# ethz-asl/TULIP

Hardware: AMD Instinct MI355X
Metric: range-images/sec training (KITTI 16->64x1024, bs=8/GPU) (higher is better)
Workload: dtype bf16; 1 GPU; tulip_base 16x1024->64x1024 training step (fwd+L1+bwd+allreduce+AdamW), per-GPU batch 8, window 2x8, patch 1x4, DropPath 0.1, reference init seed 0; global_batch=8, parallelism=dp1, hip_graph=True

## Files before the change

### include/tulip_hip.h

```cpp
#ifndef TULIP_HIP_H_
#define TULIP_HIP_H_

#include <stdint.h>

#ifdef __cplusplus
extern "C" {
#endif

#ifndef __HIP_PLATFORM_AMD__
typedef struct ihipStream_t* hipStream_t;
#endif

#define TULIP_EPI_BF16 0
#define TULIP_EPI_GELU_DUAL 1
#define TULIP_EPI_GELU_BWD 2
#define TULIP_EPI_F32 3
#define TULIP_EPI_RESID_F32 4
#define TULIP_EPI_PIXSHUF2_F32 5
#define TULIP_EPI_SPLIT_F32 7
#define TULIP_EPI_UNSHUF2_BF16 8

#define TULIP_GEMM_ACCUMULATE 1
#define TULIP_GEMM_NO_TOUCH 0x100
#define TULIP_GEMM_CHECKED 0x200
// ... 169 lines not shown
                           const float* gscale_dev, float gscale, hipStream_t stream, int in_chans, int r);
int tulip_tail_bwd_dgrad_ln_r(const uint16_t* xn, const uint16_t* We, const float* be, const float* wd, const float* dpred,
                              float* dwd_partials, int B, int H, int W, int E, const float* target, const float* gscale_dev,
                              float gscale, const float* x, const float* mean, const float* rstd, const float* gamma,
                              float* dx, uint16_t* dx_bf16, const float* cast_rowscale, int cast_rows_per_sample,
                              float* ln_partials, hipStream_t stream, int in_chans, int r);
int tulip_tail_fwd_ln_r(const float* x, const float* gamma, const float* beta, float eps, uint16_t* xn, float* mean,
                        float* rstd, const uint16_t* We, const float* be, const float* wd, float* pred, const float* target,
                        float* loss_partials, int log_transform, int B, int H, int W, int E, hipStream_t stream,
                        int in_chans, int r);
int tulip_tail_wgrad_splits_r(int B, int H, int W, int E, int in_chans, int r);
int tulip_tail_wgrad_r(const uint16_t* xn, const uint16_t* We, const float* be, const float* wd, const float* dpred,
                       float* slabs_w, float* slabs_b, int B, int H, int W, int E, const float* target,
                       const float* gscale_dev, float gscale, hipStream_t stream, int in_chans, int r);


int tulip_expand_norm_fwd(const float* y, const float* gamma, const float* beta, uint16_t* out_bf16, int ld,
                          const float* dotw, float* pred, float* mean, float* rstd, int B, int H, int W, int P, int Cn,
                          float eps, hipStream_t stream);
int tulip_expand_norm_bwd(const uint16_t* dy_fine, int ld, const float* dpred, const float* dotw, const float* y,
                          const float* mean, const float* rstd, const float* gamma, const float* beta, uint16_t* dy_nat,
                          float* partials, int B, int H, int W, int P, int Cn, hipStream_t stream);
int tulip_expand_norm_fwd_c(const float* y, const float* gamma, const float* beta, uint16_t* out_bf16, int ld,
                            const float* dotw, float* pred, float* mean, float* rstd, int B, int H, int W, int P, int Cn,
                            float eps, hipStream_t stream, int in_chans);
int tulip_expand_norm_bwd_c(const uint16_t* dy_fine, int ld, const float* dpred, const float* dotw, const float* y,
                            const float* mean, const float* rstd, const float* gamma, const float* beta, uint16_t* dy_nat,
                            float* partials, int B, int H, int W, int P, int Cn, hipStream_t stream, int in_chans);
int tulip_expand_norm_bwd_partial_rows(int B, int H, int W, int P);

int tulip_l1_loss_fwd(const float* pred, const float* target, float* partials, float* losses, int64_t n,
                      int log_transform, hipStream_t stream);
int tulip_l1_loss_bwd(const float* pred, const float* target, const float* gscale_dev, float gscale, float* dpred,
                      int64_t n, hipStream_t stream);

int tulip_adamw(float* p, float* g, float* m, float* v, uint16_t* p_bf16, int64_t n, const float* hyper,
                const uint8_t* decay_mask64, int zero_grad, hipStream_t stream);
int tulip_adamw_blocks(float* p, float* g, float* m, float* v, uint16_t* p_bf16, const int32_t* blocks, int nblocks,
                       const float* hyper, const uint8_t* decay_mask64, int zero_grad, hipStream_t stream);
int tulip_adamw_s(float* p, float* g, float* m, float* v, uint16_t* p_bf16, int64_t n, const float* hyper,
                  const uint8_t* decay_mask64, const float* lr_scale64, int zero_grad, hipStream_t stream);
int tulip_adamw_blocks_s(float* p, float* g, float* m, float* v, uint16_t* p_bf16, const int32_t* blocks, int nblocks,
                         const float* hyper, const uint8_t* decay_mask64, const float* lr_scale64, int zero_grad,
                         hipStream_t stream);

int tulip_drop_path_scales(const float* keep, float* scale, float* u_out, int nslots, int B, uint64_t seed,
                           uint64_t* counter, hipStream_t stream);

int tulip_dropout_begin(uint64_t* counter, uint64_t* key_out, int advance, hipStream_t stream);
int tulip_dropout_mask(const uint64_t* key_ptr, uint64_t seed, int site, float p, int64_t n, float* out, hipStream_t stream);
int tulip_dropout_scale(void* x, int is_bf16, int rows, int cols, int ld, const uint64_t* key_ptr, uint64_t seed, int site,
                        float p, hipStream_t stream);
int tulip_dropout_resid_ln(const float* y, const float* aux, const float* rowscale, int rows_per_sample, float* out,
                           uint16_t* out_bf16, const float* gamma, const float* beta, uint16_t* xn, float* mean, float* rstd,
                           float eps, int rows, int C, const uint64_t* key_ptr, uint64_t seed, int site, float p,
                           hipStream_t stream);
int tulip_dropout_cast(const float* dx, uint16_t* y, int rows, int cols, const float* rowscale, int rows_per_sample,
                       const uint64_t* key_ptr, uint64_t seed, int site, float p, hipStream_t stream);
int tulip_window_attn_fwd_drop(const uint16_t* qkv, const float* bias_table, const int32_t* rel_index, uint16_t* out, int B,
                               int H, int W, int C, int nh, int wh, int ww, int sh, int sw, int masked,
                               const uint64_t* key_ptr, uint64_t seed, int site, float p, hipStream_t stream);
int tulip_window_attn_bwd_drop(const uint16_t* qkv, const uint16_t* dout, const float* bias_table, const int32_t* rel_index,
                               uint16_t* dqkv, float* dbias_partials, int B, int H, int W, int C, int nh, int wh, int ww,
                               int sh, int sw, int masked, const uint64_t* key_ptr, uint64_t seed, int site, float p,
                               hipStream_t stream);

int tulip_grad_norm(const float* g, int64_t n, double* partials, const float* scale_dev, float scale, float* out,
                    hipStream_t stream);

int tulip_range_prep(const void* raw, int raw_dtype, int64_t batch_stride, int64_t row_stride, int64_t col_stride,
                     int64_t base_offset, float* hi, float* lo, int B, int H, int W, int row_factor, int col_factor,
                     int row_phase, int col_phase, float scale, int gate, float min_range, float max_range,
                     int log_transform, int roll_shift, hipStream_t stream);


int tulip_mc_aggregate(const float* preds, int passes, int64_t n, float noise_threshold, float* out,
                       hipStream_t stream);

int tulip_eval_postprocess(const float* pred, const float* hi, const float* lo, float* pred_img, float* hi_img,
                           double* partials, float* mae_out, int H, int W, int h, int w, int log_transform,
                           float gate_min, float gate_max, float keep_close, hipStream_t stream);

int tulip_range_to_xyz(const float* img, const float* sin_h, const float* cos_h, const float* sin_v,
                       const float* cos_v, float max_range, int H, int W, float* xyz, hipStream_t stream);

int tulip_range_to_xyz_durlar(const float* img, const double* col_tables, const double* row_tables,
                              const int32_t* row_offset, float max_range, float origin_offset, double z_offset, int H,
                              int W, double* xyz, hipStream_t stream);

int tulip_voxel_metrics(const void* pcd_pred, int64_t n_pred, const void* pcd_gt, int64_t n_gt, int is_f64,
                        double grid_size, uint32_t* bitmap_pred, uint32_t* bitmap_gt, int64_t bitmap_words,
                        double* scratch, double* out, hipStream_t stream);

int tulip_chamfer_sq(const void* a, int64_t na, const void* b, int64_t nb, int is_f64, float* dist_a, float* dist_b,
                     double* scratch, double* out, hipStream_t stream);

int tulip_kitti_range_map(const float* points, int64_t n, int rows, int cols, float ang_start_y, float ang_res_y,
                          float ang_res_x, float max_range, float min_range, int32_t* winner, float* out,
                          hipStream_t stream);

typedef struct tulip_swin96_desc {
    const float* x_in; float* x1; float* x_out;
    void* xn1; void* qkv; void* attn_out; void* xn2; void* fc1_pre; void* fc1_act;
    float* mean1; float* rstd1; float* mean2; float* rstd2;
    const void* w_qkv; const void* w_proj; const void* w_fc1; const void* w_fc2;
    const float* b_qkv; const float* b_proj; const float* b_fc1; const float* b_fc2;
    const float* norm1_weight; const float* norm1_bias; const float* norm2_weight; const float* norm2_bias;
    const float* bias_table; const int32_t* rel_index; const float* drop_scale_attn; const float* drop_scale_mlp;
    int B; int H; int W; int shift_h; int shift_w; int masked; float eps;
} tulip_swin96_desc;
int tulip_swin96_block_fwd(const tulip_swin96_desc* d, hipStream_t stream);
int tulip_swin96_block_fwd_profiled(const tulip_swin96_desc* d, uint64_t* stamps, hipStream_t stream);
int tulip_swin96_pair_sync_bytes(int B, int H, int W);
int tulip_swin96_pair_fwd(const tulip_swin96_desc* d0, const tulip_swin96_desc* d1, void* sync, size_t sync_bytes,
                          hipStream_t stream);

typedef struct tulip_swin96_bwd_desc {
    float* dx; const float* x_in; const float* x1;
    const void* qkv; const void* fc1_pre;
    const float* mean1; const float* rstd1; const float* mean2; const float* rstd2;
    const void* w_qkv; const void* w_proj; const void* w_fc1; const void* w_fc2;
    const float* norm1_weight; const float* norm2_weight;
    const float* bias_table; const int32_t* rel_index; const float* drop_scale_attn; const float* drop_scale_mlp;
    void* d_out_mlp; void* d_fc1_pre; void* d_out_attn; void* d_qkv;
    void* dx_bf16; const float* dx_bf16_scale;
    float* norm1_partials; float* norm2_partials; float* bias_partials;
    int B; int H; int W; int shift_h; int shift_w; int masked;
    const float* b_qkv; const float* b_fc1; const float* norm1_bias; const float* norm2_bias;
} tulip_swin96_bwd_desc;
int tulip_swin96_bwd_partial_rows(int B, int H, int W);
int tulip_swin96_block_bwd(const tulip_swin96_bwd_desc* d, hipStream_t stream);
int tulip_swin96_block_bwd_profiled(const tulip_swin96_bwd_desc* d, uint64_t* stamps, hipStream_t stream);

#define TULIP_PACK_MAX 64
typedef struct tulip_pack_item { const void* src; void* dst; int rows; int cols; int transpose; } tulip_pack_item;
int tulip_swinw_supported(int C, int H, int W);
int tulip_swinw_block_fwd(const tulip_swin96_desc* d, int C, void* out_bf16, hipStream_t stream);
int tulip_swinw_block_fwd_profiled(const tulip_swin96_desc* d, int C, void* out_bf16, uint64_t* stamps,
                                   hipStream_t stream);
int tulip_swinw_split_bytes(int C, int B, int H, int W);
int tulip_swinw_block_fwd_split(const tulip_swin96_desc* d, int C, void* out_bf16, void* exchange, size_t exchange_bytes,
                                uint64_t* stamps, hipStream_t stream);
int tulip_swinw_bwd_partial_rows(int C, int B, int H, int W);
int tulip_swinw_block_bwd(const tulip_swin96_bwd_desc* d, int C, hipStream_t stream);
int tulip_swinw_block_bwd_split(const tulip_swin96_bwd_desc* d, int C, void* exchange, size_t exchange_bytes, hipStream_t stream);
int tulip_pack_bf16_multi(const tulip_pack_item* items, int n, hipStream_t stream);

int tulip_swind_supported(int C, int H, int W, int wh, int ww);
int tulip_swind_groups(int C, int B, int H, int W, int wh, int ww);
int tulip_swind_block_fwd(const tulip_swin96_desc* d, int C, int wh, int ww, void* out_bf16, int phases, uint64_t* stamps,
                          hipStream_t stream);
int tulip_swind_block_bwd(const tulip_swin96_bwd_desc* d, int C, int wh, int ww, float* d_norm_out, int phases, uint64_t* stamps,
                          hipStream_t stream);


typedef struct tulip_merge_fwd_desc {
    const float* x; const float* gamma; const float* beta;
    const void* w_packed;
    void* xm; float* mean; float* rstd; float* y;
    void* y_bf16; int ld_bf16;
    int B, H, W, Cin; float eps;
} tulip_merge_fwd_desc;
int tulip_merge_fwd_supported(int Cin, int B, int H, int W);
int tulip_merge_fwd(const tulip_merge_fwd_desc* d, hipStream_t stream);

typedef struct tulip_merge_bwd_desc {
    const float* dx_in; const void* dy_skip; const void* w_skip_t_packed;
    void* dyb;
    const void* w_red_t_packed;
    const float* x_prev; const float* mean; const float* rstd; const float* gamma;
    float* dx_prev; float* param_partials;
    void* dx_bf16; const float* cast_rowscale; int cast_rows_per_sample;
    int B, H, W, Cp;
} tulip_merge_bwd_desc;
int tulip_merge_bwd_supported(int Cp, int B, int H, int W);
int tulip_merge_bwd_partial_rows(int Cp, int B, int H, int W);
int tulip_merge_bwd(const tulip_merge_bwd_desc* d, hipStream_t stream);

typedef struct tulip_unmerge_skip_desc {
    const void* x_bf16;
    const void* w_expand_packed; const float* b_expand;
    void* cat;
    const void* w_skip_packed; const float* b_skip;
    float* out;
    int B, H, W, C;
} tulip_unmerge_skip_desc;
int tulip_unmerge_skip_supported(int C, int B, int H, int W);
int tulip_unmerge_skip_fwd(const tulip_unmerge_skip_desc* d, hipStream_t stream);

typedef struct tulip_skip_unmerge_bwd_desc {
    const void* dy_skip; const void* w_skip_t_packed;
    void* dz;
    const void* w_expand_t_packed;
    float* dx; void* dx_bf16; const float* cast_rowscale; int cast_rows_per_sample;
    int B, H, W, C;
} tulip_skip_unmerge_bwd_desc;
int tulip_skip_unmerge_bwd(const tulip_skip_unmerge_bwd_desc* d, hipStream_t stream);

int tulip_stamp_realtime(uint64_t* dst, hipStream_t stream);
#define TULIP_ABI_VERSION 6
int tulip_abi_version(void);
const char* tulip_build_arch(void);
int tulip_dev_variants(void);

#ifdef __cplusplus
}
#endif
#endif
```

### tulip_amd/_lib.py

```python
from __future__ import annotations

import ctypes
import os
from ctypes import c_char_p, c_double, c_float, c_int, c_int64, c_void_p

_PKG = os.path.dirname(os.path.abspath(__file__))
LIB_PATH = os.environ.get("TULIP_HIP_LIB") or os.path.join(_PKG, "libtulip_hip.so")

P, I, F, L, D = c_void_p, c_int, c_float, c_int64, c_double

class Swin96Desc(ctypes.Structure):
    _fields_ = [(n, P) for n in ("x_in", "x1", "x_out", "xn1", "qkv", "attn_out", "xn2", "fc1_pre", "fc1_act", "mean1",
                                 "rstd1", "mean2", "rstd2", "w_qkv", "w_proj", "w_fc1", "w_fc2", "b_qkv", "b_proj",
                                 "b_fc1", "b_fc2", "norm1_weight", "norm1_bias", "norm2_weight", "norm2_bias",
                                 "bias_table", "rel_index", "drop_scale_attn", "drop_scale_mlp")] + \
               [(n, I) for n in ("B", "H", "W", "shift_h", "shift_w", "masked")] + [("eps", F)]


class Swin96BwdDesc(ctypes.Structure):
    _fields_ = [(n, P) for n in ("dx", "x_in", "x1", "qkv", "fc1_pre", "mean1", "rstd1", "mean2", "rstd2", "w_qkv",
                                 "w_proj", "w_fc1", "w_fc2", "norm1_weight", "norm2_weight", "bias_table", "rel_index",
                                 "drop_scale_attn", "drop_scale_mlp", "d_out_mlp", "d_fc1_pre", "d_out_attn", "d_qkv",
                                 "dx_bf16", "dx_bf16_scale", "norm1_partials", "norm2_partials", "bias_partials")] + \
               [(n, I) for n in ("B", "H", "W", "shift_h", "shift_w", "masked")] + \
               [(n, P) for n in ("b_qkv", "b_fc1", "norm1_bias", "norm2_bias")]


class ReduceRegion(ctypes.Structure):
    _fields_ = [("partials", P), ("out", P), ("stride", L), ("n", L), ("rows", I), ("overwrite", I),
                ("scatter_index", P), ("scatter_nh", I), ("scatter_len", I), ("adamw", I)]


class WgradItem(ctypes.Structure):
    _fields_ = [("dY", P), ("X", P), ("dW", P), ("db", P), ("ldy", I), ("ldx", I), ("Nw", I), ("Kw", I), ("Mtok", I),
                ("splits", I), ("overwrite", I), ("reserved_", I)]


class AdamwRef(ctypes.Structure):
    _fields_ = [(n, P) for n in ("hyper", "grad", "param", "exp_avg", "exp_avg_sq", "param_bf16", "decay_mask64")]


class DropDraw(ctypes.Structure):
    _fields_ = [("keep", P), ("scale", P), ("u_out", P), ("nslots", I), ("B", I), ("seed", ctypes.c_uint64), ("counter", P)]


class PackItem(ctypes.Structure):
    _fields_ = [("src", P), ("dst", P), ("rows", I), ("cols", I), ("transpose", I)]


class MergeFwdDesc(ctypes.Structure):
    _fields_ = [("x", P), ("gamma", P), ("beta", P), ("w_packed", P), ("xm", P), ("mean", P), ("rstd", P), ("y", P),
                ("y_bf16", P), ("ld_bf16", I), ("B", I), ("H", I), ("W", I), ("Cin", I), ("eps", F)]


class MergeBwdDesc(ctypes.Structure):
    _fields_ = [("dx_in", P), ("dy_skip", P), ("w_skip_t_packed", P), ("dyb", P), ("w_red_t_packed", P), ("x_prev", P),
                ("mean", P), ("rstd", P), ("gamma", P), ("dx_prev", P), ("param_partials", P), ("dx_bf16", P),
                ("cast_rowscale", P), ("cast_rows_per_sample", I), ("B", I), ("H", I), ("W", I), ("Cp", I)]


class UnmergeSkipDesc(ctypes.Structure):
    _fields_ = [("x_bf16", P), ("w_expand_packed", P), ("b_expand", P), ("cat", P), ("w_skip_packed", P), ("b_skip", P),
                ("out", P), ("B", I), ("H", I), ("W", I), ("C", I)]


class SkipUnmergeBwdDesc(ctypes.Structure):
    _fields_ = [("dy_skip", P), ("w_skip_t_packed", P), ("dz", P), ("w_expand_t_packed", P), ("dx", P), ("dx_bf16", P),
                ("cast_rowscale", P), ("cast_rows_per_sample", I), ("B", I), ("H", I), ("W", I), ("C", I)]


REDUCE_REGIONS_MAX, WGRAD_GROUP_MAX, PACK_MAX = 48, 16, 64
LR_GROUP_SHIFT, LR_GROUPS_MAX = 2, 64
GEMM_NO_TOUCH, GEMM_CHECKED, GEMM_NO_MID, GEMM_MID, WGRAD_SMALL_TILES, BLOCK_NO_WARM = 0x100, 0x200, 0x400, 0x800, 0x100, 8
GEMM_B_PACKED = 0x1000
ROUTE_TILE, ROUTE_FULL, ROUTE_MID, ROUTE_STREAM = range(4)
ROUTE_DEEP, ROUTE_A_TRANS, ROUTE_B_TRANS, ROUTE_FOLD, ROUTE_SPLITS_SHIFT = 0x10, 0x20, 0x40, 0x80, 8
ABI_VERSION = 6

SIGNATURES = {
    "tulip_gemm_bf16": [P, I, I, P, I, I, I, I, I, I, P, P, I, P, I, P, I, P, I, I, I, I, I, P, L, P],
    "tulip_swin96_block_fwd": [P, P],
    "tulip_swin96_pair_sync_bytes": [I, I, I],
    "tulip_swin96_pair_fwd": [P, P, P, ctypes.c_size_t, P],
    "tulip_swin96_block_bwd": [P, P],
    "tulip_swin96_block_fwd_profiled": [P, P, P],
    "tulip_swin96_block_bwd_profiled": [P, P, P],
    "tulip_swin96_bwd_partial_rows": [I, I, I],
    "tulip_swinw_supported": [I, I, I],
    "tulip_swinw_block_fwd": [P, I, P, P],
    "tulip_swinw_block_fwd_profiled": [P, I, P, P, P],
    "tulip_swinw_split_bytes": [I, I, I, I],
    "tulip_swinw_block_fwd_split": [P, I, P, P, ctypes.c_size_t, P, P],
    "tulip_swinw_bwd_partial_rows": [I, I, I, I],
    "tulip_swinw_block_bwd": [P, I, P],
    "tulip_swinw_block_bwd_split": [P, I, P, ctypes.c_size_t, P],
    "tulip_swind_supported": [I, I, I, I, I],
    "tulip_swind_groups": [I, I, I, I, I, I],
    "tulip_swind_block_fwd": [P, I, I, I, P, I, P, P],
    "tulip_swind_block_bwd": [P, I, I, I, P, I, P, P],
    "tulip_pack_bf16_multi": [P, I, P],
    "tulip_layernorm_fwd": [P, P, P, P, P, P, I, I, F, I, I, I, I, P],
    "tulip_layernorm_bwd": [P, P, P, P, P, P, P, I, I, I, I, I, I, P, P, P, I, P],
    "tulip_layernorm_bwd_splitk": [P, I, P, P, P, P, P, P, I, I, I, I, I, I, P, P, P, I, P],
    "tulip_splitk_resid_ln_supported": [I],
    "tulip_splitk_resid_ln": [P, I, I, I, P, P, I, P, I, P, I, P, I, P, P, P, P, P, F, P],
    "tulip_layernorm_bwd_partial_rows": [I, I],
    "tulip_layernorm_bwd_params": [P, P, P, P, P, P, I, I, I, I, I, I, P],
    "tulip_patch_embed_fwd": [P, P, P, P, P, P, I, I, I, I, I, I, I, I, I, F, P, I, P],
    "tulip_patch_embed_fwd_draw": [P, P, P, P, P, P, I, I, I, I, I, I, I, I, I, F, P, I, P, P],
    "tulip_patch_embed_bwd": [P, P, P, P, P, P, P, P, P, I, I, I, I, I, I, I, I, I, F, I, P],
    "tulip_patch_embed_bwd_blocks": [I],
    "tulip_window_attn_fwd": [P, P, P, P, I, I, I, I, I, I, I, I, I, I, P],
    "tulip_window_attn_bwd": [P, P, P, P, P, P, I, I, I, I, I, I, I, I, I, I, P],
    "tulip_window_attn_bwd_partial_rows": [I, I, I, I, I, I],
    "tulip_cast_f32_bf16": [P, P, I, I, P, I, P],
    "tulip_reduce_splits": [P, P, L, I, P],
    "tulip_reduce_rows2": [P, L, P, L, P, L, P, L, I, P],
    "tulip_reduce_rows_multi": [P, I, P],
    "tulip_reduce_rows_multi_adamw": [P, I, P, P],
    "tulip_wgrad_group": [P, I, P, I, P, L, I, P],
    "tulip_wgrad_tiles": [I, I, I],
    "tulip_wgrad_group_regions": [P, I, P, P, I],
    "tulip_wgrad_group_adamw": [P, I, P, I, P, L, I, P, P],
    "tulip_wgrad_group_profiled": [P, I, P, L, I, P, P],
    "tulip_gemm_effective_splits": [I, I],
    "tulip_gemm_packed_supported": [I, I, I, I],
    "tulip_gemm_route": [I, I, I, I, I, I, I, I],
    "tulip_cast_flat": [P, P, L, P],
    "tulip_cast_bf16_f32": [P, P, L, P],
    "tulip_tail_fwd": [P, P, P, P, P, I, I, I, I, P],
    "tulip_tail_bwd": [P, P, P, P, P, P, P, I, I, I, I, P, P, F, P],
    "tulip_tail_fused_bwd_supported": [I],
    "tulip_tail_bwd_dgrad": [P, P, P, P, P, P, P, I, I, I, I, P, P, F, P],
    "tulip_tail_bwd_dgrad_ln": [P, P, P, P, P, P, I, I, I, I, P, P, F, P, P, P, P, P, P, P, I, P, P],
    "tulip_tail_fwd_ln": [P, P, P, F, P, P, P, P, P, P, P, P, P, I, I, I, I, I, P],
    "tulip_l1_loss_final": [P, P, I, L, I, P],
    "tulip_tail_wgrad_splits": [I, I, I, I],
    "tulip_tail_wgrad": [P, P, P, P, P, P, P, I, I, I, I, P, P, F, P],
    "tulip_expand_norm_fwd": [P, P, P, P, I, P, P, P, P, I, I, I, I, I, F, P],
    "tulip_expand_norm_bwd": [P, I, P, P, P, P, P, P, P, P, P, I, I, I, I, I, P],
    "tulip_expand_norm_bwd_partial_rows": [I, I, I, I],
    "tulip_tail_fwd_c": [P, P, P, P, P, I, I, I, I, P, I],
    "tulip_tail_bwd_c": [P, P, P, P, P, P, P, I, I, I, I, P, P, F, P, I],
    "tulip_tail_bwd_dgrad_c": [P, P, P, P, P, P, P, I, I, I, I, P, P, F, P, I],
    "tulip_tail_bwd_dgrad_ln_c": [P, P, P, P, P, P, I, I, I, I, P, P, F, P, P, P, P, P, P, P, I, P, P, I],
    "tulip_tail_fwd_ln_c": [P, P, P, F, P, P, P, P, P, P, P, P, P, I, I, I, I, I, P, I],
    "tulip_tail_wgrad_c": [P, P, P, P, P, P, P, I, I, I, I, P, P, F, P, I],
    "tulip_tail_fwd_r": [P, P, P, P, P, I, I, I, I, P, I, I],
    "tulip_tail_bwd_r": [P, P, P, P, P, P, P, I, I, I, I, P, P, F, P, I, I],
    "tulip_tail_fused_bwd_supported_r": [I, I],
    "tulip_tail_bwd_dgrad_r": [P, P, P, P, P, P, P, I, I, I, I, P, P, F, P, I, I],
    "tulip_tail_bwd_dgrad_ln_r": [P, P, P, P, P, P, I, I, I, I, P, P, F, P, P, P, P, P, P, P, I, P, P, I, I],
    "tulip_tail_fwd_ln_r": [P, P, P, F, P, P, P, P, P, P, P, P, P, I, I, I, I, I, P, I, I],
    "tulip_tail_wgrad_splits_r": [I, I, I, I, I, I],
    "tulip_tail_wgrad_r": [P, P, P, P, P, P, P, I, I, I, I, P, P, F, P, I, I],
    "tulip_expand_norm_fwd_c": [P, P, P, P, I, P, P, P, P, I, I, I, I, I, F, P, I],
    "tulip_expand_norm_bwd_c": [P, I, P, P, P, P, P, P, P, P, P, I, I, I, I, I, P, I],
    "tulip_l1_loss_fwd": [P, P, P, P, L, I, P],
    "tulip_l1_loss_bwd": [P, P, P, F, P, L, P],
    "tulip_adamw": [P, P, P, P, P, L, P, P, I, P],
    "tulip_adamw_blocks": [P, P, P, P, P, P, I, P, P, I, P],
    "tulip_adamw_s": [P, P, P, P, P, L, P, P, P, I, P],
    "tulip_adamw_blocks_s": [P, P, P, P, P, P, I, P, P, P, I, P],
    "tulip_wgrad_group_adamw_s": [P, I, P, I, P, L, I, P, P, P],
    "tulip_reduce_rows_multi_adamw_s": [P, I, P, P, P],
    "tulip_drop_path_scales": [P, P, P, I, I, ctypes.c_uint64, P, P],
    "tulip_dropout_begin": [P, P, I, P],
    "tulip_dropout_mask": [P, ctypes.c_uint64, I, F, L, P, P],
    "tulip_dropout_scale": [P, I, I, I, I, P, ctypes.c_uint64, I, F, P],
    "tulip_dropout_resid_ln": [P, P, P, I, P, P, P, P, P, P, P, F, I, I, P, ctypes.c_uint64, I, F, P],
    "tulip_dropout_cast": [P, P, I, I, P, I, P, ctypes.c_uint64, I, F, P],
    "tulip_window_attn_fwd_drop": [P, P, P, P, I, I, I, I, I, I, I, I, I, I, P, ctypes.c_uint64, I, F, P],
    "tulip_window_attn_bwd_drop": [P, P, P, P, P, P, I, I, I, I, I, I, I, I, I, I, P, ctypes.c_uint64, I, F, P],
    "tulip_grad_norm": [P, L, P, P, F, P, P],
    "tulip_kitti_range_map": [P, L, I, I, F, F, F, F, F, P, P, P],
    "tulip_range_prep": [P, I, L, L, L, L, P, P, I, I, I, I, I, I, I, F, I, F, F, I, I, P],
    "tulip_mc_aggregate": [P, I, L, F, P, P],
    "tulip_eval_postprocess": [P, P, P, P, P, P, P, I, I, I, I, I, F, F, F, P],
    "tulip_range_to_xyz": [P, P, P, P, P, F, I, I, P, P],
    "tulip_range_to_xyz_durlar": [P, P, P, P, F, F, D, I, I, P, P],
    "tulip_voxel_metrics": [P, L, P, L, I, D, P, P, L, P, P, P],
    "tulip_chamfer_sq": [P, L, P, L, I, P, P, P, P, P],
    "tulip_merge_fwd_supported": [I, I, I, I],
    "tulip_merge_fwd": [P, P],
    "tulip_merge_bwd_supported": [I, I, I, I],
    "tulip_merge_bwd_partial_rows": [I, I, I, I],
    "tulip_merge_bwd": [P, P],
    "tulip_unmerge_skip_supported": [I, I, I, I],
    "tulip_unmerge_skip_fwd": [P, P],
    "tulip_skip_unmerge_bwd": [P, P],
    "tulip_stamp_realtime": [P, P],
    "tulip_abi_version": [],
    "tulip_build_arch": [],
    "tulip_dev_variants": [],
}

(EPI_BF16, EPI_GELU_DUAL, EPI_GELU_BWD, EPI_F32, EPI_RESID_F32, EPI_PIXSHUF2_F32, _EPI_RETIRED_6,
 EPI_SPLIT_F32, EPI_UNSHUF2_BF16) = range(9)

_lib = None


class TulipHipError(RuntimeError):
    pass


DEV_LIB_PATH = os.path.join(_PKG, "libtulip_hip_dev.so")
_libs = {}
_dev_depth = [1 if (os.environ.get("TULIP_HIP_DEV", "0") == "1" or os.environ.get("TULIP_SWIN96_RECOMPUTE", "0") != "0" or
                    os.environ.get("TULIP_SWINW_SPLIT_BWD", "0") != "0" or os.environ.get("TULIP_FC1_GRAD_WIDE", "1") == "0" or
                    os.environ.get("TULIP_FUSE_WIDE", "1") == "0") else 0]


def _open(path: str) -> ctypes.CDLL:
    if not os.path.exists(path):
        raise TulipHipError(
            f"{path} not found: build it with `python -m tulip_amd.csrc.build` "
            "(tulip_amd has no CPU or PyTorch fallback for the hot path)")
    import torch
    lib = ctypes.CDLL(path)
    for name, argtypes in SIGNATURES.items():
        try:
            fn = getattr(lib, name)
        except AttributeError as e:
            raise TulipHipError(f"symbol {name} missing from {path}") from e
        fn.argtypes = argtypes
        fn.restype = c_char_p if name == "tulip_build_arch" else c_int
    if lib.tulip_abi_version() != ABI_VERSION:
        raise TulipHipError(f"{path}: ABI version mismatch; rebuild")
    return lib


def load() -> ctypes.CDLL:
    global _lib
    path = DEV_LIB_PATH if _dev_depth[0] and not os.environ.get("TULIP_HIP_LIB") else LIB_PATH
    lib = _libs.get(path)
    if lib is None:
        lib = _libs[path] = _open(path)
    _lib = lib
    return lib


class dev_library:
    def __enter__(self):
        _dev_depth[0] += 1
        return load()

    def __exit__(self, *exc):
        _dev_depth[0] -= 1
        return False


# ... 13 lines not shown
```

### tulip_amd/csrc/swind.hip

```cpp
#ifndef TULIP_STORE_LATE_D
#define TULIP_STORE_LATE_D 1
#endif
#define TULIP_STORE_LATE TULIP_STORE_LATE_D
#include "common.h"
#include "tulip_hip.h"
#include "swin_stream.h"

namespace {

constexpr int NS = 8;

template <int C, int G>
struct GeoD {
    static constexpr int NH = C / 32, NWV = C / 128, NT = NWV * 64, T = 16 * G, KS = C / 32, HPW = NH / NS, HID = 4 * C;
    static constexpr int HS = HID / NS, KH = KS / 2, KSH = HS / 32;
    static constexpr int LPT = C / 48;
    static_assert(NWV == 2 * HPW && HS == 64 * NWV && C / 16 == 8 * NWV && (LPT == 16 || LPT == 32), "wave layout");
    static constexpr int XN_BYTES = T * C * 2;
    static constexpr int A_QX = XN_BYTES, A_QX_BYTES = HPW * 6 * G * 1024;
    static constexpr int A_HT = A_QX + A_QX_BYTES, A_HT_BYTES = HPW * 3072;
    static constexpr int A_AFF = A_HT + A_HT_BYTES;
    static constexpr int A_WARM = A_AFF + 8 * C;
    static constexpr int A_SMEM = A_WARM + 1024;
    static constexpr int B_AFF = XN_BYTES;
    static constexpr int B_WARM = B_AFF + 8 * C;
    static constexpr int B_SMEM = B_WARM + 1024;
    static constexpr int N_WARM = 2 * XN_BYTES;
    static constexpr int N_SMEM = N_WARM + 1024;
    static_assert(A_SMEM <= 163840 && N_SMEM <= 163840, "LDS");
};

struct TokMapD {
    int b, wy, wx0, H, W, wh, ww, lw, sh, sw;
    __device__ __forceinline__ void coords(int tt, int& hs, int& ws) const {
        const int t = tt & 15;
        hs = wy * wh + (t >> lw);
        ws = ((wx0 + (tt >> 4)) << lw) + (t & (ww - 1));
    }
    __device__ __forceinline__ size_t row(int tt) const {
        int hs, ws;
        coords(tt, hs, ws);
        int hh = hs + sh; if (hh >= H) hh -= H;
        int w2 = ws + sw; if (w2 >= W) w2 -= W;
        return ((size_t)b * H + hh) * W + w2;
    }
    __device__ __forceinline__ int label(int tt) const {
        int hs, ws;
        coords(tt, hs, ws);
        return 3 * region(hs, H, wh, sh) + region(ws, W, ww, sw);
    }
};
template <int G>
__device__ __forceinline__ TokMapD make_map_d(int H, int W, int wh, int ww, int sh, int sw, int grp) {
    const int nWx = W / ww, nWy = H / wh, gpr = nWx / G;
    TokMapD m;
    m.b = grp / (nWy * gpr);
    grp -= m.b * nWy * gpr;
    m.wy = grp / gpr;
    m.wx0 = (grp - m.wy * gpr) * G;
    m.H = H; m.W = W; m.wh = wh; m.ww = ww; m.lw = ww == 16 ? 4 : 3; m.sh = sh; m.sw = sw;
    return m;
}

template <int NTILE, int KSTEPS, int PF, int SEG = KSTEPS, int SEGSTRIDE = KSTEPS>
struct WS {
    bf16x8 ring[PF][NTILE];
    const bf16_t* wt[NTILE];
    static constexpr int koff(int p) { return 512 * ((p / SEG) * SEGSTRIDE + (p % SEG)); }
    __device__ __forceinline__ void start() {
        static_for<PF>([&](auto P_) {
            constexpr int p = decltype(P_)::value;
            if constexpr (p < KSTEPS) {
#pragma unroll
                for (int i = 0; i < NTILE; ++i) ring[p][i] = *(const bf16x8*)(wt[i] + koff(p));
            }
        });
    }
    template <int G, int T>
    __device__ __forceinline__ void run(f32x4 (&acc)[NTILE][G], const unsigned char* act, int t, int gq) {
        static_for<KSTEPS>([&](auto K_) {
            constexpr int ks = decltype(K_)::value;
            bf16x8 a[NTILE];
#pragma unroll
            for (int i = 0; i < NTILE; ++i) a[i] = ring[ks % PF][i];
            if constexpr (ks + PF < KSTEPS) {
#pragma unroll
                for (int i = 0; i < NTILE; ++i) ring[ks % PF][i] = *(const bf16x8*)(wt[i] + koff(ks + PF));
            }
            bf16x8 b[G];
#pragma unroll
            for (int g = 0; g < G; ++g) b[g] = frag<T>(act, ks, 16 * g + t, gq);
#pragma unroll
            for (int i = 0; i < NTILE; ++i)
#pragma unroll
                for (int g = 0; g < G; ++g) acc[i][g] = __builtin_amdgcn_mfma_f32_16x16x32_bf16(a[i], b[g], acc[i][g], 0, 0, 0);
        });
    }
};

struct SliceWarm {
    unsigned char* sink;
    int nslot, slot, ws, loff;
    bool on;
    __device__ __forceinline__ void init(int grp, int ngrp, int wid, int lane, unsigned char* lds_sink) {
        nslot = ngrp < 32 ? ngrp : 32; slot = grp; on = grp < 32;
        ws = __builtin_amdgcn_readfirstlane(wid); loff = lane * 16; sink = lds_sink;
    }
    template <int NWV>
    __device__ __forceinline__ void touch(const bf16_t* w, int nruns, int run, int stride) {
        if (!on) return;
        const int total = nruns * run;
        for (int c = slot * NWV + ws; c < total; c += nslot * NWV) {
            const int r = c / run, o = c - r * run;
            warm_touch16((const unsigned char*)(w + ((size_t)r * stride + o) * 512) + loff, sink);
        }
    }
};


struct DeepArgs {
    const float* xin; float* x1; float* xout;
    bf16_t *xn1, *qkv, *o, *xn2, *h, *g;
    float *mean1, *rstd1, *mean2, *rstd2;
    const bf16_t *wqkv, *wproj, *w1, *w2;
    const float *bqkv, *bproj, *b1, *b2, *g1, *be1, *g2, *be2;
    const float* bias_table; const int* rel_index;
    const float *ds0, *ds1;
    bf16_t* out_bf16;
    const float* dx;
    bf16_t *dyb_m, *dh, *dyb_a, *dqkv;
    float* dxn;
    float* biaspart;
    unsigned long long* prof;
    int B, H, W, wh, ww, sh, sw, masked, save, ngrp;
    float eps, scale;
};
#if TULIP_DEV_VARIANTS
#define DEEP_STAMP(k) do { if (a.prof && lane == 0) a.prof[((size_t)blockIdx.x * NWV + wid) * 16 + (k)] = __builtin_amdgcn_s_memtime(); } while (0)
#else
#define DEEP_STAMP(k) ((void)0)
#endif

template <int C, int T, int NWV>
struct RowPro {
    static constexpr int LPT = C / 48, TPW = 64 / LPT, NJ = 12, NP = (T + NWV * TPW - 1) / (NWV * TPW);
    float4 xv[NP][NJ];
    size_t row[NP];
    int tl;
    __device__ __forceinline__ int tok(int p, int wid, int lane) const { return wid * TPW + lane / LPT + p * NWV * TPW; }
    __device__ __forceinline__ void load(const float* __restrict__ x, const TokMapD& tm, int wid, int lane) {
        tl = lane % LPT;
#pragma unroll
        for (int p = 0; p < NP; ++p) {
            const int tt = tok(p, wid, lane);
            row[p] = tm.row(tt < T ? tt : T - 1);
            if (tt < T) {
#pragma unroll
                for (int j = 0; j < NJ; ++j) xv[p][j] = *(const float4*)(x + row[p] * C + 4 * tl + 4 * LPT * j);
            }
        }
    }
    __device__ __forceinline__ void layernorm(const float* aff, float eps, unsigned char* XN, bf16_t* save, float* mean, float* rstd,
                                              bool sv, int wid, int lane) {
#pragma unroll
        for (int p = 0; p < NP; ++p) {
            const int tt = tok(p, wid, lane);
            if (tt < T) {
                float sm = 0.f;
#pragma unroll
                for (int j = 0; j < NJ; ++j) sm += (xv[p][j].x + xv[p][j].y) + (xv[p][j].z + xv[p][j].w);
                const float mu = group_sum<LPT>(sm) * (1.0f / C);
                float q = 0.f;
#pragma unroll
                for (int j = 0; j < NJ; ++j) {
                    const float d0 = xv[p][j].x - mu, d1 = xv[p][j].y - mu, d2 = xv[p][j].z - mu, d3 = xv[p][j].w - mu;
                    q += (d0 * d0 + d1 * d1) + (d2 * d2 + d3 * d3);
                }
                const float rs = rsqrtf(group_sum<LPT>(q) * (1.0f / C) + eps);
                if (sv && tl == 0) { mean[row[p]] = mu; rstd[row[p]] = rs; }
#pragma unroll
                for (int j = 0; j < NJ; ++j) {
                    const int c = 4 * tl + 4 * LPT * j;
                    const float4 ga = *(const float4*)(aff + c), be = *(const float4*)(aff + C + c);
                    const bf16x4 pk = pack4((xv[p][j].x - mu) * rs * ga.x + be.x, (xv[p][j].y - mu) * rs * ga.y + be.y,
                                            (xv[p][j].z - mu) * rs * ga.z + be.z, (xv[p][j].w - mu) * rs * ga.w + be.w);
                    if (sv) store_late((bf16x4*)(save + row[p] * C + c), pk);
                    put4<T>(XN, tt, c, pk);
                }
            }
        }
    }
    __device__ __forceinline__ void scaled(float s, unsigned char* XN, bf16_t* save, bool sv, int wid, int lane) {
#pragma unroll
        for (int p = 0; p < NP; ++p) {
            const int tt = tok(p, wid, lane);
            if (tt < T) {
#pragma unroll
                for (int j = 0; j < NJ; ++j) {
                    const int c = 4 * tl + 4 * LPT * j;
                    const bf16x4 pk = pack4(xv[p][j].x * s, xv[p][j].y * s, xv[p][j].z * s, xv[p][j].w * s);
                    if (sv) store_late((bf16x4*)(save + row[p] * C + c), pk);
                    put4<T>(XN, tt, c, pk);
                }
            }
        }
    }
};

template <int C, int T, int NT>
struct RowStage {
    static constexpr int CH = C / 8, N = T * CH, NV = N / NT;
    static_assert(N % NT == 0, "chunks per thread");
    typedef unsigned u32x4_r __attribute__((ext_vector_type(4)));
    u32x4_r v[NV];
    __device__ __forceinline__ void load(const bf16_t* __restrict__ src, int ld, int col0, const TokMapD& tm, int tid) {
        static_for<NV>([&](auto K_) {
            constexpr int k = decltype(K_)::value;
            const int q = tid + k * NT, tok = q / CH, c8 = (q - tok * CH) * 8;
            v[k] = *(const u32x4_r*)(src + tm.row(tok) * ld + col0 + c8);
        });
    }
    __device__ __forceinline__ void store(unsigned char* dst, int tid) const {
        static_for<NV>([&](auto K_) {
            constexpr int k = decltype(K_)::value;
            const int q = tid + k * NT, tok = q / CH, c8 = (q - tok * CH) * 8;
            *(u32x4_r*)(dst + (c8 >> 5) * (T * 64) + tok * 64 + ((((c8 >> 3) & 3) ^ swz4(tok)) << 4)) = v[k];
        });
    }
};

template <int C, int G>
__global__ __launch_bounds__((GeoD<C, G>::NT)) void deep_attn_fwd_kernel(const DeepArgs a) {
    using Z = GeoD<C, G>;
    constexpr int T = Z::T, KS = Z::KS, KH = Z::KH, NWV = Z::NWV, HPW = Z::HPW, NH = Z::NH;
    __shared__ __attribute__((aligned(16))) unsigned char smem[Z::A_SMEM];
    unsigned char* const XN = smem;
    f32x4* const QX = (f32x4*)(smem + Z::A_QX);
    const int tid = threadIdx.x, lane = tid & 63, wid = tid >> 6, t = lane & 15, gq = lane >> 4;
    const int slice = blockIdx.x & (NS - 1), grp = blockIdx.x >> 3;
    const int hl = wid % HPW, kh = wid / HPW, head = slice * HPW + hl;
    unsigned char* const ldsV = smem + Z::A_HT + hl * 3072;
    const bool sv = a.save && slice == 0;
    const TokMapD tm = make_map_d<G>(a.H, a.W, a.wh, a.ww, a.sh, a.sw, grp);

    DEEP_STAMP(0);
    RowPro<C, T, NWV> pro;
    pro.load(a.xin, tm, wid, lane);
    const float4 affv = tid < C / 4 ? *(const float4*)(a.g1 + 4 * tid) : *(const float4*)(a.be1 + 4 * tid - C);
    WS<6, KH, 2> wq;
#pragma unroll
    for (int i = 0; i < 6; ++i) wq.wt[i] = wtile_ptr(a.wqkv, (i >> 1) * (C / 16) + 2 * head + (i & 1), C, lane) + 512 * (kh * KH);
    wq.start();
    SliceWarm warm;
    warm.init(grp, a.ngrp, wid, lane, smem + Z::A_WARM);
    warm.touch<NWV>(a.wqkv + (size_t)(2 * slice * HPW) * KS * 512, 3, 2 * HPW * KS, (C / 16) * KS);
    float* const AFF = (float*)(smem + Z::A_AFF);
    *(float4*)(AFF + 4 * tid) = affv;
    __syncthreads();
    pro.layernorm(AFF, a.eps, XN, a.xn1, a.mean1, a.rstd1, sv, wid, lane);
    size_t rows[G];
    int lab[G];
#pragma unroll
    for (int g = 0; g < G; ++g) { rows[g] = tm.row(16 * g + t); lab[g] = tm.label(16 * g + t); }
    DEEP_STAMP(1);
    __syncthreads();
    DEEP_STAMP(2);

    f32x4 acc[6][G];
    zero(acc);
    wq.template run<G, T>(acc, XN + kh * KH * (T * 64), t, gq);
    DEEP_STAMP(3);
    if (kh == 1) {
#pragma unroll
        for (int i = 0; i < 6; ++i)
#pragma unroll
            for (int g = 0; g < G; ++g) QX[((hl * 6 + i) * G + g) * 64 + lane] = acc[i][g];
    }
    __syncthreads();
    DEEP_STAMP(4);
    if (kh == 1) return;
    float rpb[4];
#pragma unroll
    for (int r = 0; r < 4; ++r) rpb[r] = a.bias_table[a.rel_index[t * 16 + gq * 4 + r] * NH + head];
    bf16x4 qkvp[6][G];
#pragma unroll
    for (int i = 0; i < 6; ++i) {
        const int n = (i >> 1) * C + 32 * head + 16 * (i & 1) + 4 * gq;
        const f32x4 bqi = ld4(a.bqkv + n);
#pragma unroll
        for (int g = 0; g < G; ++g) {
            const f32x4 s = acc[i][g] + QX[((hl * 6 + i) * G + g) * 64 + lane] + bqi;
            qkvp[i][g] = pack4(s[0], s[1], s[2], s[3]);
            if (a.save && (i & 1))
                store_bf16_tile_pair<true>(a.qkv + rows[g] * (3 * C) + n - 16 - 4 * gq, qkvp[i - 1][g], qkvp[i][g], gq);
        }
    }
#pragma unroll
    for (int g = 0; g < G; ++g) {
        const bf16x8 qf = cat8(qkvp[0][g], qkvp[1][g]);
        const bf16x8 kf = cat8(qkvp[2][g], qkvp[3][g]);
        *(bf16x4*)(ldsV + t * 64 + (4 * gq) * 2) = qkvp[4][g];
        *(bf16x4*)(ldsV + t * 64 + (16 + 4 * gq) * 2) = qkvp[5][g];
        f32x4 sc = {0.f, 0.f, 0.f, 0.f};
        if (a.masked & TULIP_ATTN_FP8) sc = __builtin_amdgcn_mfma_f32_16x16x32_fp8_fp8(bf16x8_to_fp8(kf), bf16x8_to_fp8(qf), sc, 0, 0, 0);
        else sc = __builtin_amdgcn_mfma_f32_16x16x32_bf16(kf, qf, sc, 0, 0, 0);
        float mx = -3.0e38f;
#pragma unroll
        for (int r = 0; r < 4; ++r) {
            float x = sc[r] * a.scale + rpb[r];
            if (a.masked & TULIP_ATTN_MASKED) {
                const int kl = __shfl(lab[g], gq * 4 + r, 64);
                if (kl != lab[g]) x += -100.0f;
            }
            sc[r] = x;
            mx = fmaxf(mx, x);
        }
        mx = rows_max(mx);
        float sum = 0.f;
#pragma unroll
        for (int r = 0; r < 4; ++r) { sc[r] = __expf(sc[r] - mx); sum += sc[r]; }
        sum = rows_sum(sum);
        const float inv = __builtin_amdgcn_rcpf(sum);
        const bf16x4 pb = pack4(sc[0] * inv, sc[1] * inv, sc[2] * inv, sc[3] * inv);
        bf16x4 opp[2];
#pragma unroll
        for (int dc = 0; dc < 2; ++dc) {
            const bf16x4 vt = trr(ldsV + (gq * 4 + (t >> 2)) * 64 + dc * 32 + (t & 3) * 8);
            f32x4 o = {0.f, 0.f, 0.f, 0.f};
            o = __builtin_amdgcn_mfma_f32_16x16x16bf16_1k(vt, pb, o, 0, 0, 0);
            opp[dc] = pack4(o[0], o[1], o[2], o[3]);
        }
        store_bf16_tile_pair(a.o + rows[g] * C + 32 * head, opp[0], opp[1], gq);
    }
    DEEP_STAMP(5);
}

struct NsArgs {
    const bf16_t* in; const bf16_t* w;
    const float *bias, *aux, *rowscale;
    float* out; bf16_t* out_bf16;
    unsigned long long* prof;
    int B, H, W, wh, ww, sh, sw, ngrp;
};
template <int C, int G, int KT, int EPI>
__global__ __launch_bounds__((GeoD<C, G>::NT)) void deep_nslice_kernel(const NsArgs a) {
    using Z = GeoD<C, G>;
    constexpr int T = Z::T, KS = Z::KS, NWV = Z::NWV, NT = Z::NT, NCH = KT / KS, PF = 12;
    static_assert(KT % KS == 0 && KT >= PF, "k chunks");
    __shared__ __attribute__((aligned(16))) unsigned char smem[Z::N_SMEM];
    const int tid = threadIdx.x, lane = tid & 63, wid = tid >> 6, t = lane & 15, gq = lane >> 4;
    const int slice = blockIdx.x & (NS - 1), grp = blockIdx.x >> 3;
    const TokMapD tm = make_map_d<G>(a.H, a.W, a.wh, a.ww, a.sh, a.sw, grp);
    DEEP_STAMP(0);
    RowStage<C, T, NT> st;
    st.load(a.in, 32 * KT, 0, tm, tid);
    const bf16_t* const wt = a.w + ((size_t)(slice * NWV + wid) * KT) * 512 + lane * 8;
    bf16x8 ring[PF];
#pragma unroll
    for (int p = 0; p < PF; ++p) ring[p] = *(const bf16x8*)(wt + 512 * p);
    SliceWarm warm;
    warm.init(grp, a.ngrp, wid, lane, smem + Z::N_WARM);
    warm.touch<NWV>(a.w + (size_t)(slice * NWV) * KT * 512, 1, NWV * KT, 0);
    st.store(smem, tid);
    DEEP_STAMP(1);
    __syncthreads();
    DEEP_STAMP(2);
    f32x4 acc[G];
#pragma unroll
    for (int g = 0; g < G; ++g) acc[g] = (f32x4){0.f, 0.f, 0.f, 0.f};
    static_for<NCH>([&](auto CH_) {
        constexpr int ch = decltype(CH_)::value;
        const unsigned char* const buf = smem + (ch & 1) * Z::XN_BYTES;
        if constexpr (ch + 1 < NCH) st.load(a.in, 32 * KT, (ch + 1) * C, tm, tid);
        static_for<KS>([&](auto K_) {
            constexpr int ks = decltype(K_)::value, step = ch * KS + ks;
            const bf16x8 wa = ring[step % PF];
            if constexpr (step + PF < KT) ring[step % PF] = *(const bf16x8*)(wt + 512 * (step + PF));
#pragma unroll
            for (int g = 0; g < G; ++g)
                acc[g] = __builtin_amdgcn_mfma_f32_16x16x32_bf16(wa, frag<T>(buf, ks, 16 * g + t, gq), acc[g], 0, 0, 0);
        });
        if constexpr (ch + 1 < NCH) {
            st.store(smem + ((ch + 1) & 1) * Z::XN_BYTES, tid);
            __syncthreads();
        }
    });
    DEEP_STAMP(3);
    const int c0 = slice * (C / 8) + 16 * wid + 4 * gq;
#pragma unroll
    for (int g = 0; g < G; ++g) {
        const size_t row = tm.row(16 * g + t);
        f32x4 o = acc[g];
        if constexpr (EPI == 0) {
            const float sc = a.rowscale ? a.rowscale[tm.b] : 1.0f;
            o = ld4(a.aux + row * C + c0) + sc * (o + ld4(a.bias + c0));
        }
        *(float4*)(a.out + row * C + c0) = make_float4(o[0], o[1], o[2], o[3]);
        if constexpr (EPI == 0) {
            if (a.out_bf16) *(bf16x4*)(a.out_bf16 + row * C + c0) = pack4(o[0], o[1], o[2], o[3]);
        }
    }
    DEEP_STAMP(4);
}

template <int C, int G>
__global__ __launch_bounds__((GeoD<C, G>::NT)) void deep_fc1_fwd_kernel(const DeepArgs a) {
    using Z = GeoD<C, G>;
    constexpr int T = Z::T, KS = Z::KS, NWV = Z::NWV, HID = Z::HID, HS = Z::HS;
    __shared__ __attribute__((aligned(16))) unsigned char smem[Z::B_SMEM];
    unsigned char* const XN = smem;
    const int tid = threadIdx.x, lane = tid & 63, wid = tid >> 6, t = lane & 15, gq = lane >> 4;
    const int slice = blockIdx.x & (NS - 1), grp = blockIdx.x >> 3;
    const bool sv = a.save && slice == 0;
    const TokMapD tm = make_map_d<G>(a.H, a.W, a.wh, a.ww, a.sh, a.sw, grp);
    DEEP_STAMP(0);
    RowPro<C, T, NWV> pro;
    pro.load(a.x1, tm, wid, lane);
    const float4 affv = tid < C / 4 ? *(const float4*)(a.g2 + 4 * tid) : *(const float4*)(a.be2 + 4 * tid - C);
    WS<4, KS, 3> w1s;
#pragma unroll
    for (int i = 0; i < 4; ++i) w1s.wt[i] = wtile_ptr(a.w1, slice * (HS / 16) + 4 * wid + i, C, lane);
    w1s.start();
    SliceWarm warm;
    warm.init(grp, a.ngrp, wid, lane, smem + Z::B_WARM);
    warm.touch<NWV>(a.w1 + (size_t)(slice * (HS / 16)) * KS * 512, 1, (HS / 16) * KS, 0);
    float* const AFF = (float*)(smem + Z::B_AFF);
    *(float4*)(AFF + 4 * tid) = affv;
    __syncthreads();
    pro.layernorm(AFF, a.eps, XN, a.xn2, a.mean2, a.rstd2, sv, wid, lane);
    size_t rows[G];
#pragma unroll
    for (int g = 0; g < G; ++g) rows[g] = tm.row(16 * g + t);
    DEEP_STAMP(1);
    __syncthreads();
    DEEP_STAMP(2);
    f32x4 acc[4][G];
    zero(acc);
    w1s.template run<G, T>(acc, XN, t, gq);
    DEEP_STAMP(3);
    bf16x4 hprev[G], gprev[G];
#pragma unroll
    for (int i = 0; i < 4; ++i) {
        const int n = slice * HS + 64 * wid + 16 * i + 4 * gq;
        const f32x4 bb = ld4(a.b1 + n);
#pragma unroll
        for (int g = 0; g < G; ++g) {
            bf16x4 hp = pack4(acc[i][g][0] + bb[0], acc[i][g][1] + bb[1], acc[i][g][2] + bb[2], acc[i][g][3] + bb[3]);
            const f32x2 h01 = {bf2f((bf16_t)hp[0]), bf2f((bf16_t)hp[1])}, h23 = {bf2f((bf16_t)hp[2]), bf2f((bf16_t)hp[3])};
            f32x2 g01, g23;
            if (a.save) {
                f32x2 d01, d23;
                gelu_exact_and_grad2(h01, g01, d01);
                gelu_exact_and_grad2(h23, g23, d23);
                hp = pack4(d01.x, d01.y, d23.x, d23.y);
            } else {
                g01 = gelu_exact2(h01); g23 = gelu_exact2(h23);
            }
            const bf16x4 gp = pack4(g01.x, g01.y, g23.x, g23.y);
            if (i & 1) {
                const size_t off = rows[g] * HID + slice * HS + 64 * wid + 16 * (i - 1);
                store_bf16_tile_pair(a.g + off, gprev[g], gp, gq);
                if (a.save) store_bf16_tile_pair<true>(a.h + off, hprev[g], hp, gq);
            } else {
                hprev[g] = hp; gprev[g] = gp;
            }
        }
    }
    DEEP_STAMP(4);
}

template <int C, int G>
__global__ __launch_bounds__((GeoD<C, G>::NT)) void deep_fc2_bwd_kernel(const DeepArgs a) {
    using Z = GeoD<C, G>;
    constexpr int T = Z::T, KS = Z::KS, NWV = Z::NWV, HID = Z::HID, HS = Z::HS;
    __shared__ __attribute__((aligned(16))) unsigned char smem[Z::B_SMEM];
    unsigned char* const DY = smem;
    const int tid = threadIdx.x, lane = tid & 63, wid = tid >> 6, t = lane & 15, gq = lane >> 4;
    const int slice = blockIdx.x & (NS - 1), grp = blockIdx.x >> 3;
    const TokMapD tm = make_map_d<G>(a.H, a.W, a.wh, a.ww, a.sh, a.sw, grp);
    const float s1v = a.ds1 ? a.ds1[tm.b] : 1.0f;
    DEEP_STAMP(0);
    RowPro<C, T, NWV> pro;
    pro.load(a.dx, tm, wid, lane);
    WS<4, KS, 3> w2s;
#pragma unroll
    for (int i = 0; i < 4; ++i) w2s.wt[i] = wtile_ptr(a.w2, slice * (HS / 16) + 4 * wid + i, C, lane);
    w2s.start();
    SliceWarm warm;
    warm.init(grp, a.ngrp, wid, lane, smem + Z::B_WARM);
    warm.touch<NWV>(a.w2 + (size_t)(slice * (HS / 16)) * KS * 512, 1, (HS / 16) * KS, 0);
    pro.scaled(s1v, DY, a.dyb_m, slice == 0, wid, lane);
    size_t rows[G];
#pragma unroll
    for (int g = 0; g < G; ++g) rows[g] = tm.row(16 * g + t);
    DEEP_STAMP(1);
    __syncthreads();
    DEEP_STAMP(2);
    f32x4 acc[4][G];
    zero(acc);
    w2s.template run<G, T>(acc, DY, t, gq);
    DEEP_STAMP(3);
    bf16x4 hv[4][G];
#pragma unroll
    for (int i = 0; i < 4; ++i)
#pragma unroll
        for (int g = 0; g < G; ++g)
            hv[i][g] = ld_saved((const bf16x4*)(a.h + rows[g] * HID + slice * HS + 64 * wid + 16 * i + 4 * gq));
    bf16x4 dprev[G];
#pragma unroll
    for (int i = 0; i < 4; ++i) {
#pragma unroll
        for (int g = 0; g < G; ++g) {
            const bf16x4 dp = pack4(acc[i][g][0] * bf2f((bf16_t)hv[i][g][0]), acc[i][g][1] * bf2f((bf16_t)hv[i][g][1]),
                                    acc[i][g][2] * bf2f((bf16_t)hv[i][g][2]), acc[i][g][3] * bf2f((bf16_t)hv[i][g][3]));
            if (i & 1) store_bf16_tile_pair(a.dh + rows[g] * HID + slice * HS + 64 * wid + 16 * (i - 1), dprev[g], dp, gq);
            else dprev[g] = dp;
        }
    }
    DEEP_STAMP(4);
}

template <int C, int G>
__global__ __launch_bounds__((GeoD<C, G>::NT)) void deep_attn_bwd_kernel(const DeepArgs a) {
    using Z = GeoD<C, G>;
    constexpr int T = Z::T, KS = Z::KS, KH = Z::KH, NWV = Z::NWV, HPW = Z::HPW, NH = Z::NH, NT = Z::NT;
    __shared__ __attribute__((aligned(16))) unsigned char smem[Z::A_SMEM];
    unsigned char* const DY = smem;
    f32x4* const PX = (f32x4*)(smem + Z::A_QX);
    const int tid = threadIdx.x, lane = tid & 63, wid = tid >> 6, t = lane & 15, gq = lane >> 4;
    const int slice = blockIdx.x & (NS - 1), grp = blockIdx.x >> 3;
    const int hl = wid % HPW, kh = wid / HPW, head = slice * HPW + hl;
    const TokMapD tm = make_map_d<G>(a.H, a.W, a.wh, a.ww, a.sh, a.sw, grp);
    DEEP_STAMP(0);
    RowStage<C, T, NT> st;
    st.load(a.dyb_a, C, 0, tm, tid);
    WS<2, KH, 6> wps;
#pragma unroll
    for (int i = 0; i < 2; ++i) wps.wt[i] = wtile_ptr(a.wproj, 2 * head + i, C, lane) + 512 * (kh * KH);
    wps.start();
    SliceWarm warm;
    warm.init(grp, a.ngrp, wid, lane, smem + Z::A_WARM);
    warm.touch<NWV>(a.wproj + (size_t)(2 * slice * HPW) * KS * 512, 1, 2 * HPW * KS, 0);
    st.store(DY, tid);
    size_t rows[G];
    int lab[G];
#pragma unroll
    for (int g = 0; g < G; ++g) { rows[g] = tm.row(16 * g + t); lab[g] = tm.label(16 * g + t); }
    DEEP_STAMP(1);
    __syncthreads();
    DEEP_STAMP(2);
    f32x4 acc[2][G];
    zero(acc);
    wps.template run<G, T>(acc, DY + kh * KH * (T * 64), t, gq);
    DEEP_STAMP(3);
    if (kh == 1) {
#pragma unroll
        for (int i = 0; i < 2; ++i)
#pragma unroll
            for (int g = 0; g < G; ++g) PX[((hl * 2 + i) * G + g) * 64 + lane] = acc[i][g];
    }
    __syncthreads();
    DEEP_STAMP(4);
    if (kh == 1) return;
    float bias_q[4], bias_k[4];
#pragma unroll
    for (int r = 0; r < 4; ++r) {
        bias_q[r] = a.bias_table[a.rel_index[t * 16 + gq * 4 + r] * NH + head];
        bias_k[r] = a.bias_table[a.rel_index[(gq * 4 + r) * 16 + t] * NH + head];
    }
    bf16x4 dop[2][G];
#pragma unroll
    for (int i = 0; i < 2; ++i)
#pragma unroll
        for (int g = 0; g < G; ++g) {
            const f32x4 s = acc[i][g] + PX[((hl * 2 + i) * G + g) * 64 + lane];
            dop[i][g] = pack4(s[0], s[1], s[2], s[3]);
        }
    bf16x4 qkvr[6][G];
#pragma unroll
    for (int i = 0; i < 6; ++i)
#pragma unroll
        for (int g = 0; g < G; ++g)
            qkvr[i][g] = ld_saved((const bf16x4*)(a.qkv + rows[g] * (3 * C) + (i >> 1) * C + 32 * head + 16 * (i & 1) + 4 * gq));
    unsigned char* ldsQ = smem + Z::A_HT + hl * 3072;
    unsigned char* ldsK = ldsQ + 1024;
    unsigned char* ldsD = ldsK + 1024;
    const f32x4 z = {0.f, 0.f, 0.f, 0.f};
    const int troff = (gq * 4 + (t >> 2)) * 64 + (t & 3) * 8;
    float bsum[4] = {0.f, 0.f, 0.f, 0.f};
#pragma unroll
    for (int g = 0; g < G; ++g) {
        bf16x8 qf = cat8(qkvr[0][g], qkvr[1][g]), kf = cat8(qkvr[2][g], qkvr[3][g]);
        if (a.masked & TULIP_ATTN_FP8) { qf = round_through_fp8(qf); kf = round_through_fp8(kf); }
        const bf16x8 vf = cat8(qkvr[4][g], qkvr[5][g]);
        const bf16x8 df = cat8(dop[0][g], dop[1][g]);
        const int o0 = t * 64 + (4 * gq) * 2, o1 = t * 64 + (16 + 4 * gq) * 2;
        *(bf16x4*)(ldsQ + o0) = __builtin_shufflevector(qf, qf, 0, 1, 2, 3);  *(bf16x4*)(ldsQ + o1) = __builtin_shufflevector(qf, qf, 4, 5, 6, 7);
        *(bf16x4*)(ldsK + o0) = __builtin_shufflevector(kf, kf, 0, 1, 2, 3);  *(bf16x4*)(ldsK + o1) = __builtin_shufflevector(kf, kf, 4, 5, 6, 7);
        *(bf16x4*)(ldsD + o0) = dop[0][g];   *(bf16x4*)(ldsD + o1) = dop[1][g];
        f32x4 sq = __builtin_amdgcn_mfma_f32_16x16x32_bf16(kf, qf, z, 0, 0, 0);
        f32x4 sk = __builtin_amdgcn_mfma_f32_16x16x32_bf16(qf, kf, z, 0, 0, 0);
        f32x4 dpq = __builtin_amdgcn_mfma_f32_16x16x32_bf16(vf, df, z, 0, 0, 0);
        f32x4 dpk = __builtin_amdgcn_mfma_f32_16x16x32_bf16(df, vf, z, 0, 0, 0);
        float mx = -3.0e38f;
#pragma unroll
        for (int r = 0; r < 4; ++r) {
            float xq = sq[r] * a.scale + bias_q[r];
            float xk = sk[r] * a.scale + bias_k[r];
            if (a.masked & TULIP_ATTN_MASKED) {
                const int ol = __shfl(lab[g], gq * 4 + r, 64);
                if (ol != lab[g]) { xq += -100.0f; xk += -100.0f; }
            }
            sq[r] = xq; sk[r] = xk;
            mx = fmaxf(mx, xq);
        }
        mx = rows_max(mx);
        float sum = 0.f;
#pragma unroll
        for (int r = 0; r < 4; ++r) sum += __expf(sq[r] - mx);
        sum = rows_sum(sum);
        const float lse = mx + __logf(sum);
        float pq[4], pk[4], delta = 0.f;
#pragma unroll
        for (int r = 0; r < 4; ++r) {
            pq[r] = __expf(sq[r] - lse);
            pk[r] = __expf(sk[r] - __shfl(lse, gq * 4 + r, 64));
            delta += pq[r] * dpq[r];
        }
        delta = rows_sum(delta);
        float dsq[4], dsk[4];
#pragma unroll
        for (int r = 0; r < 4; ++r) {
            dsq[r] = pq[r] * (dpq[r] - delta);
            dsk[r] = pk[r] * (dpk[r] - __shfl(delta, gq * 4 + r, 64));
            bsum[r] += dsq[r];
        }
        const bf16x4 dsq_b = pack4(dsq[0], dsq[1], dsq[2], dsq[3]);
        const bf16x4 dsk_b = pack4(dsk[0], dsk[1], dsk[2], dsk[3]);
        const bf16x4 pk_b = pack4(pk[0], pk[1], pk[2], pk[3]);
        bf16x4 oprev[3];
#pragma unroll
        for (int dc = 0; dc < 2; ++dc) {
            const bf16x4 kt = trr(ldsK + troff + dc * 32);
            const bf16x4 qt = trr(ldsQ + troff + dc * 32);
            const bf16x4 dt = trr(ldsD + troff + dc * 32);
            const f32x4 dq = __builtin_amdgcn_mfma_f32_16x16x16bf16_1k(kt, dsq_b, z, 0, 0, 0);
            const f32x4 dk = __builtin_amdgcn_mfma_f32_16x16x16bf16_1k(qt, dsk_b, z, 0, 0, 0);
            const f32x4 dv = __builtin_amdgcn_mfma_f32_16x16x16bf16_1k(dt, pk_b, z, 0, 0, 0);
            const bf16x4 o[3] = {pack4(dq[0] * a.scale, dq[1] * a.scale, dq[2] * a.scale, dq[3] * a.scale),
                                 pack4(dk[0] * a.scale, dk[1] * a.scale, dk[2] * a.scale, dk[3] * a.scale),
                                 pack4(dv[0], dv[1], dv[2], dv[3])};
#pragma unroll
            for (int sec = 0; sec < 3; ++sec) {
                if (dc) store_bf16_tile_pair(a.dqkv + rows[g] * (3 * C) + sec * C + 32 * head, oprev[sec], o[sec], gq);
                else oprev[sec] = o[sec];
            }
        }
    }
    *(float4*)(a.biaspart + (size_t)grp * (NH * 256) + head * 256 + t * 16 + gq * 4) = make_float4(bsum[0], bsum[1], bsum[2], bsum[3]);
    DEEP_STAMP(5);
}

inline int deep_g(int C, int B, int H, int W, int wh, int ww) {
    const int windows = B * (H / wh) * (W / ww), nWx = W / ww;
    if (C == 768 && nWx % 2 == 0 && windows / 2 >= 32) return 2;
    return 1;
}
inline bool deep_ok(int C, int B, int H, int W, int wh, int ww) {
    return (C == 768 || C == 1536) && B > 0 && H > 0 && W > 0 && ((wh == 2 && ww == 8) || (wh == 1 && ww == 16)) && H % wh == 0 &&
           W % ww == 0;
}

template <int C, int G>
int launch_deep(const DeepArgs& a, int which, hipStream_t stream) {
    const dim3 grid(a.ngrp * NS), block(GeoD<C, G>::NT);
    switch (which) {
        case 0: hipLaunchKernelGGL((deep_attn_fwd_kernel<C, G>), grid, block, 0, stream, a); break;
        case 1: hipLaunchKernelGGL((deep_fc1_fwd_kernel<C, G>), grid, block, 0, stream, a); break;
        case 2: hipLaunchKernelGGL((deep_fc2_bwd_kernel<C, G>), grid, block, 0, stream, a); break;
        default: hipLaunchKernelGGL((deep_attn_bwd_kernel<C, G>), grid, block, 0, stream, a); break;
    }
    TULIP_CHECK_LAUNCH();
    return TULIP_OK;
}
int dispatch_deep(const DeepArgs& a, int C, int G, int which, hipStream_t stream) {
    if (C == 768) return G == 2 ? launch_deep<768, 2>(a, which, stream) : launch_deep<768, 1>(a, which, stream);
    return launch_deep<1536, 1>(a, which, stream);
}
template <int C, int G>
int launch_ns(const NsArgs& a, int ksec, int epi, hipStream_t stream) {
    const dim3 grid(a.ngrp * NS), block(GeoD<C, G>::NT);
    constexpr int KS = C / 32;
    if (epi == 0 && ksec == 1) hipLaunchKernelGGL((deep_nslice_kernel<C, G, KS, 0>), grid, block, 0, stream, a);
    else if (epi == 0 && ksec == 4) hipLaunchKernelGGL((deep_nslice_kernel<C, G, 4 * KS, 0>), grid, block, 0, stream, a);
    else if (epi == 1 && ksec == 4) hipLaunchKernelGGL((deep_nslice_kernel<C, G, 4 * KS, 1>), grid, block, 0, stream, a);
    else if (epi == 1 && ksec == 3) hipLaunchKernelGGL((deep_nslice_kernel<C, G, 3 * KS, 1>), grid, block, 0, stream, a);
    else return TULIP_ERR_ARG;
    TULIP_CHECK_LAUNCH();
    return TULIP_OK;
}
int dispatch_ns(const NsArgs& a, int C, int G, int ksec, int epi, hipStream_t stream) {
    if (C == 768) return G == 2 ? launch_ns<768, 2>(a, ksec, epi, stream) : launch_ns<768, 1>(a, ksec, epi, stream);
    return launch_ns<1536, 1>(a, ksec, epi, stream);
}

}

extern "C" int tulip_swind_supported(int C, int H, int W, int wh, int ww) { return deep_ok(C, 1, H, W, wh, ww) ? 1 : 0; }

extern "C" int tulip_swind_groups(int C, int B, int H, int W, int wh, int ww) {
    if (!deep_ok(C, B, H, W, wh, ww)) return 0;
    return B * (H / wh) * (W / ww) / deep_g(C, B, H, W, wh, ww);
}

extern "C" int tulip_swind_block_fwd(const tulip_swin96_desc* d, int C, int wh, int ww, void* out_bf16, int phases, uint64_t* stamps,
                                     hipStream_t stream) {
    if (!d || !deep_ok(C, d->B, d->H, d->W, wh, ww) || d->shift_h < 0 || d->shift_h >= d->H || d->shift_w < 0 || d->shift_w >= d->W ||
        !(phases & 15))
        return TULIP_ERR_ARG;
    const bool any = d->xn1 || d->qkv || d->xn2 || d->fc1_pre || d->mean1 || d->rstd1 || d->mean2 || d->rstd2;
    const bool all = d->xn1 && d->qkv && d->xn2 && d->fc1_pre && d->mean1 && d->rstd1 && d->mean2 && d->rstd2;
    if ((any && !all) || !d->x1 || !d->attn_out || !d->fc1_act || !d->x_in || !d->x_out) return TULIP_ERR_ARG;
    if (all && !(d->masked & TULIP_BLOCK_FC1_GRAD)) return TULIP_ERR_ARG;
    DeepArgs a = {};
    const int G = deep_g(C, d->B, d->H, d->W, wh, ww);
    a.ngrp = d->B * (d->H / wh) * (d->W / ww) / G;
    a.xin = d->x_in; a.x1 = d->x1; a.xout = d->x_out;
    a.xn1 = (bf16_t*)d->xn1; a.qkv = (bf16_t*)d->qkv; a.o = (bf16_t*)d->attn_out; a.xn2 = (bf16_t*)d->xn2;
    a.h = (bf16_t*)d->fc1_pre; a.g = (bf16_t*)d->fc1_act;
    a.mean1 = d->mean1; a.rstd1 = d->rstd1; a.mean2 = d->mean2; a.rstd2 = d->rstd2;
    a.wqkv = (const bf16_t*)d->w_qkv; a.wproj = (const bf16_t*)d->w_proj; a.w1 = (const bf16_t*)d->w_fc1; a.w2 = (const bf16_t*)d->w_fc2;
    a.bqkv = d->b_qkv; a.bproj = d->b_proj; a.b1 = d->b_fc1; a.b2 = d->b_fc2;
    a.g1 = d->norm1_weight; a.be1 = d->norm1_bias; a.g2 = d->norm2_weight; a.be2 = d->norm2_bias;
    a.bias_table = d->bias_table; a.rel_index = d->rel_index; a.ds0 = d->drop_scale_attn; a.ds1 = d->drop_scale_mlp;
    a.out_bf16 = (bf16_t*)out_bf16;
    a.prof = (unsigned long long*)stamps;
#if !TULIP_DEV_VARIANTS
    if (stamps) return TULIP_ERR_NOT_BUILT;
#endif
    a.B = d->B; a.H = d->H; a.W = d->W; a.wh = wh; a.ww = ww; a.sh = d->shift_h; a.sw = d->shift_w; a.masked = d->masked;
    a.save = all ? 1 : 0;
    a.eps = d->eps; a.scale = 0.17677669529663687f;
    NsArgs n = {};
    n.B = a.B; n.H = a.H; n.W = a.W; n.wh = wh; n.ww = ww; n.sh = a.sh; n.sw = a.sw; n.ngrp = a.ngrp;
    const size_t pstride = (size_t)a.ngrp * NS * (C / 128) * 16;
    int rc;
    if (phases & 1) { if ((rc = dispatch_deep(a, C, G, 0, stream))) return rc; }
    if (phases & 2) {
        n.in = a.o; n.w = a.wproj; n.bias = a.bproj; n.aux = a.xin; n.rowscale = a.ds0; n.out = a.x1; n.out_bf16 = nullptr;
        n.prof = a.prof ? a.prof + pstride : nullptr;
        if ((rc = dispatch_ns(n, C, G, 1, 0, stream))) return rc;
    }
    if (phases & 4) {
        DeepArgs b = a;
        if (b.prof) b.prof += 2 * pstride;
        if ((rc = dispatch_deep(b, C, G, 1, stream))) return rc;
    }
    if (phases & 8) {
        n.in = a.g; n.w = a.w2; n.bias = a.b2; n.aux = a.x1; n.rowscale = a.ds1; n.out = a.xout; n.out_bf16 = a.out_bf16;
        n.prof = a.prof ? a.prof + 3 * pstride : nullptr;
        if ((rc = dispatch_ns(n, C, G, 4, 0, stream))) return rc;
    }
    return TULIP_OK;
}

extern "C" int tulip_swind_block_bwd(const tulip_swin96_bwd_desc* d, int C, int wh, int ww, float* d_norm_out, int phases,
                                     uint64_t* stamps, hipStream_t stream) {
    if (!d || !deep_ok(C, d->B, d->H, d->W, wh, ww) || d->shift_h < 0 || d->shift_h >= d->H || d->shift_w < 0 || d->shift_w >= d->W ||
        !(phases & 15) || !(d->masked & TULIP_BLOCK_FC1_GRAD) || !d->qkv || !d->fc1_pre || !d_norm_out)
        return TULIP_ERR_ARG;
    DeepArgs a = {};
    const int G = deep_g(C, d->B, d->H, d->W, wh, ww);
    a.ngrp = d->B * (d->H / wh) * (d->W / ww) / G;
    a.dx = d->dx;
    a.qkv = (bf16_t*)d->qkv; a.h = (bf16_t*)d->fc1_pre;
    a.wqkv = (const bf16_t*)d->w_qkv; a.wproj = (const bf16_t*)d->w_proj; a.w1 = (const bf16_t*)d->w_fc1; a.w2 = (const bf16_t*)d->w_fc2;
    a.bias_table = d->bias_table; a.rel_index = d->rel_index; a.ds0 = d->drop_scale_attn; a.ds1 = d->drop_scale_mlp;
    a.dyb_m = (bf16_t*)d->d_out_mlp; a.dh = (bf16_t*)d->d_fc1_pre; a.dyb_a = (bf16_t*)d->d_out_attn; a.dqkv = (bf16_t*)d->d_qkv;
    a.dxn = d_norm_out; a.biaspart = d->bias_partials;
    a.prof = (unsigned long long*)stamps;
#if !TULIP_DEV_VARIANTS
    if (stamps) return TULIP_ERR_NOT_BUILT;
#endif
    a.B = d->B; a.H = d->H; a.W = d->W; a.wh = wh; a.ww = ww; a.sh = d->shift_h; a.sw = d->shift_w; a.masked = d->masked;
    a.save = 1;
    a.scale = 0.17677669529663687f;
    NsArgs n = {};
    n.B = a.B; n.H = a.H; n.W = a.W; n.wh = wh; n.ww = ww; n.sh = a.sh; n.sw = a.sw; n.ngrp = a.ngrp;
    n.out = a.dxn;
    const size_t pstride = (size_t)a.ngrp * NS * (C / 128) * 16;
    int rc;
    if (phases & 1) { if ((rc = dispatch_deep(a, C, G, 2, stream))) return rc; }
    if (phases & 2) {
        n.in = a.dh; n.w = a.w1; n.prof = a.prof ? a.prof + pstride : nullptr;
        if ((rc = dispatch_ns(n, C, G, 4, 1, stream))) return rc;
    }
    if (phases & 4) {
        DeepArgs b = a;
        if (b.prof) b.prof += 2 * pstride;
        if ((rc = dispatch_deep(b, C, G, 3, stream))) return rc;
    }
    if (phases & 8) {
        n.in = a.dqkv; n.w = a.wqkv; n.prof = a.prof ? a.prof + 3 * pstride : nullptr;
        if ((rc = dispatch_ns(n, C, G, 3, 1, stream))) return rc;
    }
    return TULIP_OK;
}
```

### tulip_amd/engine.py

```python
from __future__ import annotations

import math
import os
from dataclasses import dataclass, field
from typing import Dict, List, Optional, Tuple

import torch

from . import knobs, ops
from ._lib import (EPI_BF16, EPI_F32, EPI_GELU_BWD, EPI_GELU_DUAL, EPI_PIXSHUF2_F32, EPI_RESID_F32,
                   EPI_UNSHUF2_BF16,
                   EPI_SPLIT_F32)

ALIGN = 64


def _ceil(a: int, b: int) -> int:
    return (a + b - 1) // b * b


def effective_window(H: int, window, shift: bool):
    wh, ww = int(window[0]), int(window[1])
    L = wh * ww
    if H < wh:
# ... 367 lines not shown
                                    for b in range(m.depths[s])])
        self.n_drop_slots = slot
        self._drop_mods = []
        for sp in self.blocks:
            blk = m.get_submodule(sp.prefix)
            self._drop_mods.append((blk.attn.attn_drop, blk.attn.proj_drop, blk.mlp.drop1, blk.mlp.drop2))
        self._drop = ()
        self._keep = None
        self._pending = []
        self._side_dirty = False
        self._graphs = {}
        self._rel32 = None

    def hidden(self, C: int) -> int:
        return int(C * self.model.mlp_ratio)

    def invalidate(self):
        self.params = None
        self.plans.clear()
        self._graphs.clear()

    def bind(self, device):
        self._cur_params = None
        if self.params is not None and self.device == device:
            self._cur_params = self.params.current_params(self.model)
            if self._cur_params is not None:
                return
        self.device = device
        self.plans.clear()
        self._graphs.clear()
        self.params = FlatParams(self.model, device)
        by_width: Dict[int, List[str]] = {}
        if self.fuse_wide or self.fuse_wide_bwd or self.fuse_deep:
            for sp in self.blocks:
                if self._fusable_wide(sp) or self._fusable_deep(sp):
                    by_width.setdefault(sp.C, []).extend(sp.prefix + suffix for suffix in (
                        ".attn.qkv.weight", ".attn.proj.weight", ".mlp.fc1.weight", ".mlp.fc2.weight"))
        if self.fuse_glue and self.model.patch_unmerging:
            m, nl = self.model, self.model.num_layers
            glue = [f"layers.{s}.downsample.reduction.weight" for s in range(nl - 1)]
            glue += [f"skip_connection_layers.{i}.weight" for i in range(nl - 1)]
            glue += [f"layers_up.{i}.upsample.expand.weight" for i in range(nl - 2)]
            if nl > 1:
                glue.append("first_patch_expanding.expand.weight")
            def ok(n):
                r, c = self.params.shape[n][0], self.params.shape[n][1]
                if n.endswith("reduction.weight"):
                    return c // 4 in (96, 192, 384)
                if n.startswith("skip_connection_layers."):
                    return r in (96, 192, 384)
                return c in (192, 384, 768)
            by_width[0] = [n for n in glue if n in self.params.offset and ok(n)]
        self.params.make_packed(by_width, with_transposes=self.fuse_wide_bwd or self.fuse_deep or bool(by_width.get(0)))
        self.params.pk_active = {w for w in by_width if w < 768 and by_width[w]}
        rel = self.model.layers[0].blocks[0].attn.relative_position_index
        self._rel32 = rel.to(device=device, dtype=torch.int32).contiguous()
        rates = torch.ones(max(1, self.n_drop_slots), 1)
        for sp in self.blocks:
            if sp.slot >= 0:
                rates[sp.slot] = rates[sp.slot + 1] = 1.0 - sp.rate
        self._keep = rates.to(device)
        self.early_flush = frozenset(sp.prefix for sp in self.enc_blocks[0][:1])
        self._drop_seed = torch.initial_seed()
        self._drop_counter = torch.zeros(1, dtype=torch.int64, device=device)

    def plan(self, B: int) -> Plan:
        if B not in self.plans:
            self.plans[B] = Plan(self, B)
            widths = {sp.C for sp in self.blocks if ((self.fuse_wide or self.fuse_wide_bwd) and self._fusable_wide(sp, B))
                      or self._fusable_deep(sp, B)}
            if not widths <= self.params.pk_active:
                self.params.pk_active |= widths
                self.params.pack_epoch += 1
                self._pack_mark_tag_ = None
                if not self.params.shadow_dirty:
                    self.params.refresh_transposes()
        if getattr(self, "_ws", None) is None or self._ws.device != self.device:
            self._ws = torch.empty(self.WS_ELEMS + (1 << 20), dtype=torch.float32, device=self.device)
            self._ws_ptr = self._ws.data_ptr()
            self._ws_side = torch.empty(self.WS_ELEMS + (1 << 20), dtype=torch.float32, device=self.device)
            self._ws_side_ptr = self._ws_side.data_ptr()
            self._side_stream = torch.cuda.Stream(device=self.device)
        return self.plans[B]

    def draw_drop_scales(self, P: Plan, train: bool, drop_u: Optional[torch.Tensor] = None):
        self._pending_draw = None
        if not train or self.n_drop_slots == 0:
            P.drop_scale.fill_(1.0)
            return
        if drop_u is None:
            self._pending_draw = (P, (self._keep, P.drop_scale, P.drop_u, self.n_drop_slots, P.B, self._drop_seed, self._drop_counter))
            return
        P.drop_u.copy_(drop_u)
        torch.floor(self._keep + P.drop_u, out=P.drop_scale)
        P.drop_scale.div_(self._keep)

    _pending_draw = None

    def _ds(self, P: Plan, sp: BlockSpec, branch: int):
        if sp.slot < 0:
            return None
        return P.drop_scale.data_ptr() + 4 * (sp.slot + branch) * P.B

    infer_no_save = True
    _no_save = False
    fuse_block96 = knobs.on("TULIP_FUSE_BLOCK96", True)
    fuse_block96_bwd = knobs.on("TULIP_FUSE_BLOCK96_BWD", True)

    recompute96 = knobs.on("TULIP_SWIN96_RECOMPUTE", False)
    fc1_grad96 = knobs.on("TULIP_FC1_GRAD", True)

    def _hgrad96(self, sp: BlockSpec) -> bool:
        return (self.fc1_grad96 and self.fuse_block96 and self.fuse_block96_bwd and self._fusable96(sp)
                and not self._recomp96(sp))

    fc1_grad_wide = knobs.on("TULIP_FC1_GRAD_WIDE", True)

    def _hgrad_wide(self, sp: BlockSpec, B: int) -> bool:
        return self.fc1_grad_wide and self.fuse_wide and self.fuse_wide_bwd and self._fusable_wide(sp, B)

    def _recomp96(self, sp: BlockSpec) -> bool:
        return self.recompute96 and self.fuse_block96 and self.fuse_block96_bwd and self._fusable96(sp)

    def _fusable96(self, sp: BlockSpec) -> bool:
        return (sp.C == 96 and sp.nh == 3 and self.hidden(sp.C) == 384 and tuple(sp.win) == (2, 8) and sp.W % 64 == 0
                and sp.H % 2 == 0)

    attn_fp8 = knobs.is_one("TULIP_ATTN_FP8")

    def check_attn_fp8(self):
        if self.attn_fp8 and self.win_len != 16:
            raise NotImplementedError(f"tulip_amd: fp8 attention scores (TULIP_ATTN_FP8=1 / Trainer(attn_fp8=True)) are built for "
                                      f"16-token windows only; this model's window {self.window} has {self.win_len} tokens")

    def _mask_arg(self, sp: BlockSpec, B: Optional[int] = None) -> int:
        hg = self._hgrad96(sp) or (B is not None and (self._hgrad_wide(sp, B) or self._fusable_deep(sp, B)))
        return int(bool(sp.shift)) | (2 if self.attn_fp8 else 0) | (4 if hg else 0) | (8 if self.no_warm else 0)

    split_wide = knobs.on("TULIP_SWINW_SPLIT", True)
    split_wide_bwd = knobs.on("TULIP_SWINW_SPLIT_BWD", False)
    fuse_wide = knobs.on("TULIP_FUSE_WIDE", True)
    fuse_wide_bwd = knobs.on("TULIP_FUSE_WIDE_BWD", True)
    wide_widths = (192, 384)
    wide_min_windows = knobs.integer("TULIP_FUSE_WIDE_MIN_WINDOWS", 128)

    def _fusable_wide(self, sp: BlockSpec, B: Optional[int] = None) -> bool:
        ok = (sp.C in self.wide_widths and sp.C in (192, 384) and sp.nh * 32 == sp.C and self.hidden(sp.C) == 4 * sp.C
              and tuple(sp.win) == (2, 8) and sp.W % 16 == 0 and sp.H % 2 == 0)
        if ok and B is not None and sp.C == 384:
            ok = B * (sp.H // 2) * (sp.W // 8) >= self.wide_min_windows
        return ok

    fuse_deep = knobs.on("TULIP_FUSE_DEEP", True)
    deep_min_windows = knobs.integer("TULIP_FUSE_DEEP_MIN_WINDOWS", 32)
    deep_max_windows = knobs.integer("TULIP_FUSE_DEEP_MAX_WINDOWS", 64)

    def _fusable_deep(self, sp: BlockSpec, B: Optional[int] = None) -> bool:
        ok = (self.fuse_deep and sp.C in (768, 1536) and sp.nh * 32 == sp.C and self.hidden(sp.C) == 4 * sp.C
              and tuple(sp.win) in ((2, 8), (1, 16)) and sp.H % sp.win[0] == 0 and sp.W % sp.win[1] == 0)
        if ok and B is not None:
            ok = self.deep_min_windows <= B * (sp.H // sp.win[0]) * (sp.W // sp.win[1]) <= self.deep_max_windows
        return ok

    def _fused_bwd(self, sp: BlockSpec, B: int) -> bool:
        if self._dblock(sp):
            return False
        return ((self.fuse_block96_bwd and self._fusable96(sp)) or (self.fuse_wide_bwd and self._fusable_wide(sp, B))
                or self._fusable_deep(sp, B))

    fuse_splitk_ln = True
    fuse_tail_bwd = True
    fuse_tail_ln_bwd = True
    _tail_fused = False

    def _unfused(self, sp: BlockSpec, B: int) -> bool:
        if self._dblock(sp):
            return True
        return not ((self.fuse_wide and self._fusable_wide(sp, B)) or (self.fuse_block96 and self._fusable96(sp))
                    or self._fusable_deep(sp, B))

    def dropout_state(self) -> tuple:
        act = lambda d: float(d.p) if (d.training and d.p > 0.0) else 0.0
        blocks = tuple(tuple(act(d) for d in mods) for mods in self._drop_mods)
        pos = act(self.model.pos_drop)
        if pos == 0.0 and not any(any(b) for b in blocks):
            return ()
        return (pos, blocks)

    def _dblock(self, sp: BlockSpec) -> bool:
        return bool(self._drop) and any(self._drop[1][sp.idx])

    def _dp(self, sp: BlockSpec, kind: int) -> float:
        return self._drop[1][sp.idx][kind] if self._drop else 0.0

    def _dkw(self, P: Plan, sp: Optional[BlockSpec], kind: int) -> dict:
        site = 0 if sp is None else 1 + 4 * sp.idx + kind
        p = self._drop[0] if sp is None else self._dp(sp, kind)
        return dict(key=P.drop_key, seed=self._drop_seed, site=site, p=p)

    def _gemm_resid_ln(self, A, Wt, M, N, K, *, lda, ldb, bias, out, aux, rowscale, tok, ln, out2=None):
        gamma, beta, xn, mean, rstd = ln
        gn = (N + 95) // 96
        blocks = ((M + 63) // 64) * gn if ((M + 127) // 128) * gn < 256 else ((M + 127) // 128) * gn
        s = 1
        if self.fuse_splitk_ln and blocks <= 96 and K >= 768 and ops.splitk_resid_ln_supported(N):
            s = ops.gemm_effective_splits(K, max(1, min(256 // blocks, K // 256, (self.WS_ELEMS * 4) // (M * N * 4))))
        if s > 1:
            ops.gemm(A, Wt, M, N, K, lda=lda, ldb=ldb, epi=EPI_SPLIT_F32, out=self._ws_ptr, ldo=N, splits=s)
            ops.splitk_resid_ln(self._ws_ptr, s, M, N, bias, aux, N, rowscale, tok, out, N, out2, N if out2 is not None else 0,
                                gamma, beta, xn, mean, rstd, self.eps)
            return
        self._gemm(A, Wt, M, N, K, lda=lda, ldb=ldb, epi=EPI_RESID_F32, bias=bias, out=out, aux=aux, ldaux=N,
                   rowscale=rowscale, rows_per_sample=tok, out2=out2, ldo2=N if out2 is not None else 0)
        ops.layernorm_fwd(out, gamma, beta, xn, mean, rstd, M, N, self.eps)

    def _block_fwd(self, P: Plan, sp: BlockSpec, xin, xout, out_bf16=None, ln1_done=False, next_sp=None):
        W_ = self.params
        p = sp.prefix
        B, C, nh = P.B, sp.C, sp.nh
        M, Hd, tok = B * sp.H * sp.W, self.hidden(sp.C), sp.H * sp.W
        drop = self._dblock(sp)
        wide = self.fuse_wide and self._fusable_wide(sp, B) and not drop
        if self._fusable_deep(sp, B) and not drop:
            self._join_pack(p)
            keep = (".o", ".x1", ".g")
            sv = (lambda k: P[p + k] if k in keep else None) if self._no_save else (lambda k: P[p + k])
            wf = W_.p16p
            ops.swind_block_fwd(
                C, sp.win, out_bf16=out_bf16,
                x_in=xin, x1=sv(".x1"), x_out=xout, xn1=sv(".xn1"), qkv=sv(".qkv"), attn_out=sv(".o"),
                xn2=sv(".xn2"), fc1_pre=sv(".h"), fc1_act=sv(".g"), mean1=sv(".mean1"),
                rstd1=sv(".rstd1"), mean2=sv(".mean2"), rstd2=sv(".rstd2"),
                w_qkv=wf(p + ".attn.qkv.weight"), w_proj=wf(p + ".attn.proj.weight"),
                w_fc1=wf(p + ".mlp.fc1.weight"), w_fc2=wf(p + ".mlp.fc2.weight"),
                b_qkv=W_.p32(p + ".attn.qkv.bias"), b_proj=W_.p32(p + ".attn.proj.bias"),
                b_fc1=W_.p32(p + ".mlp.fc1.bias"), b_fc2=W_.p32(p + ".mlp.fc2.bias"),
                norm1_weight=W_.p32(p + ".norm1.weight"), norm1_bias=W_.p32(p + ".norm1.bias"),
                norm2_weight=W_.p32(p + ".norm2.weight"), norm2_bias=W_.p32(p + ".norm2.bias"),
                bias_table=W_.p32(p + ".attn.relative_position_bias_table"), rel_index=self._rel32,
                drop_scale_attn=self._ds(P, sp, 0), drop_scale_mlp=self._ds(P, sp, 1), B=B, H=sp.H, W=sp.W,
                shift_h=sp.sft[0], shift_w=sp.sft[1], masked=self._mask_arg(sp, B), eps=self.eps)
            return
        if wide or (self.fuse_block96 and self._fusable96(sp) and not drop):
            if wide:
                self._join_pack(p)
            xkw = {}
            if wide and self.split_wide and (self._no_save or self._hgrad_wide(sp, B)):
                nb = ops.swinw_split_bytes(C, B, sp.H, sp.W)
                if nb:
                    P.scratch("xchg." + p, (nb + 3) // 4)
                    xkw["exchange"] = P.bufs["xchg." + p]
            launch = (lambda **kw: ops.swinw_block_fwd(C, out_bf16=out_bf16, **xkw, **kw)) if wide else ops.swin96_block_fwd
            wf = W_.p16p if wide else W_.p16
            lean = (not wide) and self._recomp96(sp)
            sv = (lambda k: None) if self._no_save else (lambda k: None if (lean and k in (".qkv", ".h")) else P[p + k])
            launch(
                x_in=xin, x1=sv(".x1"), x_out=xout, xn1=sv(".xn1"), qkv=sv(".qkv"), attn_out=sv(".o"),
                xn2=sv(".xn2"), fc1_pre=sv(".h"), fc1_act=sv(".g"), mean1=sv(".mean1"),
                rstd1=sv(".rstd1"), mean2=sv(".mean2"), rstd2=sv(".rstd2"),
                w_qkv=wf(p + ".attn.qkv.weight"), w_proj=wf(p + ".attn.proj.weight"),
                w_fc1=wf(p + ".mlp.fc1.weight"), w_fc2=wf(p + ".mlp.fc2.weight"),
                b_qkv=W_.p32(p + ".attn.qkv.bias"), b_proj=W_.p32(p + ".attn.proj.bias"),
                b_fc1=W_.p32(p + ".mlp.fc1.bias"), b_fc2=W_.p32(p + ".mlp.fc2.bias"),
                norm1_weight=W_.p32(p + ".norm1.weight"), norm1_bias=W_.p32(p + ".norm1.bias"),
                norm2_weight=W_.p32(p + ".norm2.weight"), norm2_bias=W_.p32(p + ".norm2.bias"),
                bias_table=W_.p32(p + ".attn.relative_position_bias_table"), rel_index=self._rel32,
                drop_scale_attn=self._ds(P, sp, 0), drop_scale_mlp=self._ds(P, sp, 1), B=B, H=sp.H, W=sp.W,
                shift_h=sp.sft[0], shift_w=sp.sft[1], masked=self._mask_arg(sp, B), eps=self.eps)
            if out_bf16 is not None and not wide:
                ops.cast_f32_bf16(xout, out_bf16, M, C)
            return
        if not ln1_done:
            ops.layernorm_fwd(xin, W_.p32(p + ".norm1.weight"), W_.p32(p + ".norm1.bias"), P[p + ".xn1"],
                              P[p + ".mean1"], P[p + ".rstd1"], M, C, self.eps)
        self._gemm(P[p + ".xn1"], W_.p16(p + ".attn.qkv.weight"), M, 3 * C, C, lda=C, ldb=C, epi=EPI_BF16,
                 bias=W_.p32(p + ".attn.qkv.bias"), out=P[p + ".qkv"])
        if drop:
            self._block_fwd_drop(P, sp, xin, xout, out_bf16, next_sp)
            return
        ops.window_attn_fwd(P[p + ".qkv"], W_.p32(p + ".attn.relative_position_bias_table"), self._rel32, P[p + ".o"],
                            B, sp.H, sp.W, C, nh, sp.win, sp.sft, self._mask_arg(sp))
        self._gemm_resid_ln(P[p + ".o"], W_.p16(p + ".attn.proj.weight"), M, C, C, lda=C, ldb=C,
                            bias=W_.p32(p + ".attn.proj.bias"), out=P[p + ".x1"], aux=xin, rowscale=self._ds(P, sp, 0), tok=tok,
                            ln=(W_.p32(p + ".norm2.weight"), W_.p32(p + ".norm2.bias"), P[p + ".xn2"], P[p + ".mean2"],
                                P[p + ".rstd2"]))
        self._gemm(P[p + ".xn2"], W_.p16(p + ".mlp.fc1.weight"), M, Hd, C, lda=C, ldb=C, epi=EPI_GELU_DUAL,
                 bias=W_.p32(p + ".mlp.fc1.bias"), out=P[p + ".h"], out2=P[p + ".g"], ldo2=Hd)
        if next_sp is not None:
            q = next_sp.prefix
            self._gemm_resid_ln(P[p + ".g"], W_.p16(p + ".mlp.fc2.weight"), M, C, Hd, lda=Hd, ldb=Hd,
                                bias=W_.p32(p + ".mlp.fc2.bias"), out=xout, aux=P[p + ".x1"], rowscale=self._ds(P, sp, 1),
                                tok=tok, out2=out_bf16,
                                ln=(W_.p32(q + ".norm1.weight"), W_.p32(q + ".norm1.bias"), P[q + ".xn1"], P[q + ".mean1"],
                                    P[q + ".rstd1"]))
            return
        self._gemm(P[p + ".g"], W_.p16(p + ".mlp.fc2.weight"), M, C, Hd, lda=Hd, ldb=Hd, epi=EPI_RESID_F32,
                 bias=W_.p32(p + ".mlp.fc2.bias"), out=xout, aux=P[p + ".x1"], ldaux=C,
                 rowscale=self._ds(P, sp, 1), rows_per_sample=tok, out2=out_bf16, ldo2=C if out_bf16 is not None else 0)

    def _block_fwd_drop(self, P: Plan, sp: BlockSpec, xin, xout, out_bf16, next_sp):
        W_ = self.params
        p = sp.prefix
        B, C, nh = P.B, sp.C, sp.nh
        M, Hd, tok = B * sp.H * sp.W, self.hidden(sp.C), sp.H * sp.W
        if self._dp(sp, 0):
            ops.window_attn_fwd_drop(P[p + ".qkv"], W_.p32(p + ".attn.relative_position_bias_table"), self._rel32, P[p + ".o"],
# ... 475 lines not shown
                    if sp > 1 and gbias is not None:
                        self.adam_sites[gbias] = "fold"
                grp.append(ops.wgrad_item(dY, ldy, X, ldx, Nw, Kw, Mtok, gout, gbias, sp, overwrite=self.grad_overwrite,
                                          adamw=step_here))
                items.pop(0)
            room = _lib.REDUCE_REGIONS_MAX - 2 * len(grp)
            extra, regions = regions[:room], regions[room:]
            ops.wgrad_group(grp, extra, ws, ws_bytes, adam=self._adam_arg(), small_tiles=self.wgrad_small_tiles)
        while regions:
            ops.reduce_rows_multi(regions[:_lib.REDUCE_REGIONS_MAX], adam=self._adam_arg())
            regions = regions[_lib.REDUCE_REGIONS_MAX:]
        for fn in fns:
            fn()

    def _flush_wgrads(self, advance: bool = True, mark: bool = False):
        st, ws = self._side_stream, self._ws_side_ptr
        if not self._pending:
            if mark:
                self._mark_side()
            return
        main = torch.cuda.current_stream()
        if advance:
            self._release_deferred()
            ev = torch.cuda.Event()
            ev.record(main)
            self._deferred = (ev, st, ws, self._pending, mark)
            self._pending = []
            self._side_dirty = True
            return
        st.wait_stream(main)
        with torch.cuda.stream(st):
            self._issue_pending(ws)
        if mark:
            self._pack_ev = torch.cuda.Event()
            self._pack_ev.record(st)
        self._pending = []
        self._side_dirty = True

    _deferred = None
    pack_at_end = False
    _pack_ev = None

    @property
    def _pack_mark_tag(self):
        t = getattr(self, "_pack_mark_tag_", None)
        if t is None:
            W_ = self.params
            last = -1
            for n in W_.packed_names():
                if n not in W_.pk_late:
                    last = max(last, next(k for k, (_, end) in enumerate(W_.groups) if W_.offset[n] < end))
            t = self._pack_mark_tag_ = W_.groups[last][0] if last >= 0 else ""
        return t

    def _mark_side(self):
        self._release_deferred()
        self._side_stream.wait_stream(torch.cuda.current_stream())
        self._pack_ev = torch.cuda.Event()
        self._pack_ev.record(self._side_stream)
        self._side_dirty = True

    def _release_deferred(self):
        d, self._deferred = self._deferred, None
        if d is None:
            return
        ev, st, ws, pending, mark = d
        st.wait_event(ev)
        with torch.cuda.stream(st):
            self._issue_pending(ws, pending)
        if mark:
            self._pack_ev = torch.cuda.Event()
            self._pack_ev.record(st)

    detach_buckets = False
    _detached = None

    def take_detached(self):
        d, self._detached = self._detached, None
        return d

    def issue_detached(self, pending, ws: int):
        self._issue_pending(ws, pending)
        if self._carry:
            carry, self._carry = list(self._carry), ()
            ops.reduce_rows_multi(carry, adam=self._adam_arg())

    def _wait_side(self):
        self._release_deferred()
        self._flush_carry()
        if getattr(self, "_side_dirty", False):
            torch.cuda.current_stream().wait_stream(self._side_stream)
            self._side_dirty = False

    def _join_side(self):
        self._flush_wgrads()
        self._release_deferred()
        self._flush_carry()
        if getattr(self, "_side_dirty", False):
            torch.cuda.current_stream().wait_stream(self._side_stream)
            self._side_dirty = False

    def _wgrad_launch(self, dY, ldy, X, ldx, Nw, Kw, Mtok, gout, gbias, ws):
        splits = self._splits(Nw, Kw, Mtok)
        if splits == 1:
            ops.gemm(dY, X, Nw, Kw, Mtok, lda=ldy, ldb=ldx, a_trans=True, b_trans=True, epi=EPI_F32, out=gout, ldo=Kw,
                     accumulate=True, out2=gbias)
            return
        wsb = ws + 4 * splits * Nw * Kw if gbias is not None else None
        ops.gemm(dY, X, Nw, Kw, Mtok, lda=ldy, ldb=ldx, a_trans=True, b_trans=True, epi=EPI_SPLIT_F32, out=ws, ldo=Kw,
                 splits=splits, out2=wsb)
        ops.reduce_rows2(ws, Nw * Kw, gout, Nw * Kw, wsb, Nw, gbias, Nw if gbias is not None else 0, splits)

    def _dgrad_ln_bwd(self, P: Plan, dY, Wt, M, C, K, dxn, ln_args, ln_kw):
        gn = (C + 95) // 96
        blocks = ((M + 63) // 64) * gn if ((M + 127) // 128) * gn < 256 else ((M + 127) // 128) * gn
        s = 1
        if self.fuse_splitk_ln and blocks <= 96 and K >= 768 and ops.layernorm_bwd_partial_rows(M, C) > 0:
            s = ops.gemm_effective_splits(K, max(1, min(256 // blocks, K // 256, (self.WS_ELEMS * 4) // (M * C * 4))))
        if s > 1:
            ops.gemm(dY, Wt, M, C, K, lda=K, ldb=C, b_trans=True, epi=EPI_SPLIT_F32, out=self._ws_ptr, ldo=C, splits=s)
            self._ln_bwd(P, None, *ln_args, slabs=(self._ws_ptr, s), **ln_kw)
            return
        self._gemm(dY, Wt, M, C, K, lda=K, ldb=C, b_trans=True, epi=EPI_BF16, out=dxn, ldo=C)
        self._ln_bwd(P, dxn, *ln_args, **ln_kw)

    def _ln_bwd(self, P: Plan, dy, x, mean, rstd, gamma, dres, dx, rows, C, gw, gb, tag, merge=False, H=0, W=0,
                cast=None, slabs=None):
        cb, cs, ct = cast if cast is not None else (None, None, 1)
        nrows = ops.layernorm_bwd_partial_rows(rows, C)
        if nrows == 0:
            if self.grad_overwrite:
                g0 = self._gflat.data_ptr()
                for ptr in (gw, gb):
                    self._gflat[(ptr - g0) // 4:(ptr - g0) // 4 + C].zero_()
            ops.layernorm_bwd_params(dy, x, mean, rstd, gw, gb, rows, C, merge=merge, B=P.B, H=H, W=W)
            ops.layernorm_bwd(dy, x, mean, rstd, gamma, dres, dx, rows, C, merge=merge, B=P.B, H=H, W=W,
                              dx_bf16=cb, cast_rowscale=cs, cast_rows_per_sample=ct)
            return
        part = P.scratch("lnp." + tag, nrows * 2 * C)
        if slabs is not None:
            ops.layernorm_bwd_splitk(slabs[0], slabs[1], x, mean, rstd, gamma, dres, dx, rows, C, merge=merge, B=P.B, H=H,
                                     W=W, param_partials=part, dx_bf16=cb, cast_rowscale=cs, cast_rows_per_sample=ct)
        else:
            ops.layernorm_bwd(dy, x, mean, rstd, gamma, dres, dx, rows, C, merge=merge, B=P.B, H=H, W=W,
                              param_partials=part, dx_bf16=cb, cast_rowscale=cs, cast_rows_per_sample=ct)
        self._fold(part, 2 * C, gw, C, nrows)
        self._fold(part + 4 * C, 2 * C, gb, C, nrows)

    def _mlp_cast(self, P: Plan, sp: BlockSpec):
        if self._fused_bwd(sp, P.B) or self._dblock(sp):
            return None
        return (P[sp.prefix + ".dyb_m"], self._ds(P, sp, 1), sp.H * sp.W)

    def _block_bwd(self, P: Plan, sp: BlockSpec, xin, dx, G, have_dyb=False, next_cast=None):
        W_ = self.params
        p = sp.prefix
        B, C, nh = P.B, sp.C, sp.nh
        M, Hd, tok = B * sp.H * sp.W, self.hidden(sp.C), sp.H * sp.W
        dxn, dO, dh, dqkv = P["t.dxn"], P["t.do"], P[p + ".dh"], P[p + ".dqkv"]
        dyb = P[p + ".dyb_m"]
        drop = self._dblock(sp)
        if self._fusable_deep(sp, B) and not drop:
            dn = P.scratch("deep.dxn", max(P.B * q.H * q.W * q.C for q in self.blocks if self._fusable_deep(q, P.B)))
            R = ops.swind_groups(C, B, sp.H, sp.W, sp.win)
            apart = P.scratch("apart." + p, R * nh * self.win_len ** 2)
            wt = W_.p16t
            desc = dict(
                dx=dx, x_in=xin, x1=P[p + ".x1"], qkv=P[p + ".qkv"], fc1_pre=P[p + ".h"], mean1=P[p + ".mean1"],
                rstd1=P[p + ".rstd1"], mean2=P[p + ".mean2"], rstd2=P[p + ".rstd2"],
                w_qkv=wt(p + ".attn.qkv.weight"), w_proj=wt(p + ".attn.proj.weight"),
                w_fc1=wt(p + ".mlp.fc1.weight"), w_fc2=wt(p + ".mlp.fc2.weight"),
                norm1_weight=W_.p32(p + ".norm1.weight"), norm2_weight=W_.p32(p + ".norm2.weight"),
                bias_table=W_.p32(p + ".attn.relative_position_bias_table"), rel_index=self._rel32,
                drop_scale_attn=self._ds(P, sp, 0), drop_scale_mlp=self._ds(P, sp, 1), d_out_mlp=dyb, d_fc1_pre=dh,
                d_out_attn=P[p + ".dyb_a"], d_qkv=dqkv, bias_partials=apart, B=B, H=sp.H, W=sp.W, shift_h=sp.sft[0],
                shift_w=sp.sft[1], masked=self._mask_arg(sp, B))
            ops.swind_block_bwd(C, sp.win, dn, phases=3, **desc)
            self._release_deferred()
            self._wgrad(dyb, C, P[p + ".g"], Hd, C, Hd, M, G(p + ".mlp.fc2.weight"), G(p + ".mlp.fc2.bias"))
            self._wgrad(dh, Hd, P[p + ".xn2"], C, Hd, C, M, G(p + ".mlp.fc1.weight"), G(p + ".mlp.fc1.bias"))
            self._ln_bwd(P, None, P[p + ".x1"], P[p + ".mean2"], P[p + ".rstd2"], W_.p32(p + ".norm2.weight"), dx, dx, M, C,
                         G(p + ".norm2.weight"), G(p + ".norm2.bias"), p + ".2", cast=(P[p + ".dyb_a"], self._ds(P, sp, 0), tok),
                         slabs=(dn, 1))
            ops.swind_block_bwd(C, sp.win, dn, phases=12, **desc)
            self._wgrad(P[p + ".dyb_a"], C, P[p + ".o"], C, C, C, M, G(p + ".attn.proj.weight"), G(p + ".attn.proj.bias"))
            self._fold_bias_table(P, p, apart, R, nh, G(p + ".attn.relative_position_bias_table"))
            self._ln_bwd(P, None, xin, P[p + ".mean1"], P[p + ".rstd1"], W_.p32(p + ".norm1.weight"), dx, dx, M, C,
                         G(p + ".norm1.weight"), G(p + ".norm1.bias"), p + ".1", cast=next_cast, slabs=(dn, 1))
            self._wgrad(dqkv, 3 * C, P[p + ".xn1"], C, 3 * C, C, M, G(p + ".attn.qkv.weight"), G(p + ".attn.qkv.bias"))
            if self._lagged_hook is not None:
                fn, self._lagged_hook = self._lagged_hook, None
                fn()
            return
        if self._fused_bwd(sp, B):
            wide = not (self.fuse_block96_bwd and self._fusable96(sp))
            cb, cs, ct = next_cast if next_cast is not None else (None, None, tok)
            if cs is not None and ct != tok:
                raise ValueError("fused block backward: the cast scale must be per sample")
            R = ops.swinw_bwd_partial_rows(C, B, sp.H, sp.W) if wide else ops.swin96_bwd_partial_rows(B, sp.H, sp.W)
            ln1, ln2 = P.scratch("lnp." + p + ".1", R * 2 * C), P.scratch("lnp." + p + ".2", R * 2 * C)
            apart = P.scratch("apart." + p, R * nh * self.win_len ** 2)
            xkw = {}
            if wide and self.split_wide_bwd and self._hgrad_wide(sp, B):
                nb = ops.swinw_split_bytes(C, B, sp.H, sp.W)
                if nb:
                    P.scratch("xchg." + p, (nb + 3) // 4)
                    xkw["exchange"] = P.bufs["xchg." + p]
            launch = (lambda **kw: ops.swinw_block_bwd(C, **xkw, **kw)) if wide else ops.swin96_block_bwd
            wt = W_.p16t if wide else W_.p16
            lean = (not wide) and self._recomp96(sp)
            extra = dict(b_qkv=W_.p32(p + ".attn.qkv.bias"), b_fc1=W_.p32(p + ".mlp.fc1.bias"),
                         norm1_bias=W_.p32(p + ".norm1.bias"), norm2_bias=W_.p32(p + ".norm2.bias")) if lean else {}
            launch(
                dx=dx, x_in=xin, x1=P[p + ".x1"], qkv=None if lean else P[p + ".qkv"], fc1_pre=None if lean else P[p + ".h"],
                mean1=P[p + ".mean1"],
                rstd1=P[p + ".rstd1"], mean2=P[p + ".mean2"], rstd2=P[p + ".rstd2"],
                w_qkv=wt(p + ".attn.qkv.weight"), w_proj=wt(p + ".attn.proj.weight"),
                w_fc1=wt(p + ".mlp.fc1.weight"), w_fc2=wt(p + ".mlp.fc2.weight"),
                norm1_weight=W_.p32(p + ".norm1.weight"), norm2_weight=W_.p32(p + ".norm2.weight"),
                bias_table=W_.p32(p + ".attn.relative_position_bias_table"), rel_index=self._rel32,
                drop_scale_attn=self._ds(P, sp, 0), drop_scale_mlp=self._ds(P, sp, 1), d_out_mlp=dyb, d_fc1_pre=dh,
                d_out_attn=P[p + ".dyb_a"], d_qkv=dqkv, dx_bf16=cb, dx_bf16_scale=cs, norm1_partials=ln1,
                norm2_partials=ln2, bias_partials=apart, B=B, H=sp.H, W=sp.W, shift_h=sp.sft[0], shift_w=sp.sft[1],
                masked=self._mask_arg(sp, B), **extra)
            self._release_deferred()
            self._wgrad(dyb, C, P[p + ".g"], Hd, C, Hd, M, G(p + ".mlp.fc2.weight"), G(p + ".mlp.fc2.bias"))
            self._wgrad(dh, Hd, P[p + ".xn2"], C, Hd, C, M, G(p + ".mlp.fc1.weight"), G(p + ".mlp.fc1.bias"))
            self._wgrad(P[p + ".dyb_a"], C, P[p + ".o"], C, C, C, M, G(p + ".attn.proj.weight"), G(p + ".attn.proj.bias"))
            self._wgrad(dqkv, 3 * C, P[p + ".xn1"], C, 3 * C, C, M, G(p + ".attn.qkv.weight"), G(p + ".attn.qkv.bias"))
            self._fold(ln2, 2 * C, G(p + ".norm2.weight"), C, R)
            self._fold(ln2 + 4 * C, 2 * C, G(p + ".norm2.bias"), C, R)
            self._fold(ln1, 2 * C, G(p + ".norm1.weight"), C, R)
            self._fold(ln1 + 4 * C, 2 * C, G(p + ".norm1.bias"), C, R)
            self._fold_bias_table(P, p, apart, R, nh, G(p + ".attn.relative_position_bias_table"))
            if self._lagged_hook is not None:
                fn, self._lagged_hook = self._lagged_hook, None
                fn()
            return
        if drop and self._dp(sp, 3):
            ops.dropout_cast(dx, dyb, M, C, self._ds(P, sp, 1), tok, **self._dkw(P, sp, 3))
        elif not have_dyb or drop:
            ops.cast_f32_bf16(dx, dyb, M, C, self._ds(P, sp, 1), tok)
        self._gemm(dyb, W_.p16(p + ".mlp.fc2.weight"), M, Hd, C, lda=C, ldb=Hd, b_trans=True, epi=EPI_GELU_BWD, out=dh,
                 ldo=Hd, aux=P[p + ".h"], ldaux=Hd)
        if drop and self._dp(sp, 2):
            ops.dropout_scale(dh, True, M, Hd, **self._dkw(P, sp, 2))
        self._release_deferred()
        self._wgrad(dyb, C, P[p + ".g"], Hd, C, Hd, M, G(p + ".mlp.fc2.weight"), G(p + ".mlp.fc2.bias"))
        self._dgrad_ln_bwd(P, dh, W_.p16(p + ".mlp.fc1.weight"), M, C, Hd, dxn,
                           (P[p + ".x1"], P[p + ".mean2"], P[p + ".rstd2"], W_.p32(p + ".norm2.weight"), dx, dx, M, C,
                            G(p + ".norm2.weight"), G(p + ".norm2.bias"), p + ".2"),
                           dict(cast=None if (drop and self._dp(sp, 1)) else (P[p + ".dyb_a"], self._ds(P, sp, 0), tok)))
        if drop and self._dp(sp, 1):
            ops.dropout_cast(dx, P[p + ".dyb_a"], M, C, self._ds(P, sp, 0), tok, **self._dkw(P, sp, 1))
        self._wgrad(dh, Hd, P[p + ".xn2"], C, Hd, C, M, G(p + ".mlp.fc1.weight"), G(p + ".mlp.fc1.bias"))
        if sp.prefix in self.early_flush:
            self._flush_wgrads(advance=False)
        dyb = P[p + ".dyb_a"]
        self._gemm(dyb, W_.p16(p + ".attn.proj.weight"), M, C, C, lda=C, ldb=C, b_trans=True, epi=EPI_BF16, out=dO,
                 ldo=C)
        self._wgrad(dyb, C, P[p + ".o"], C, C, C, M, G(p + ".attn.proj.weight"), G(p + ".attn.proj.bias"))
        R = ops.window_attn_bwd_partial_rows(B, sp.H, sp.W, nh, sp.win)
        apart = P.scratch("apart." + p, R * nh * self.win_len ** 2)
        if drop and self._dp(sp, 0):
            ops.window_attn_bwd_drop(P[p + ".qkv"], dO, W_.p32(p + ".attn.relative_position_bias_table"), self._rel32, dqkv,
                                     apart, B, sp.H, sp.W, C, nh, sp.win, sp.sft, self._mask_arg(sp), **self._dkw(P, sp, 0))
        else:
            ops.window_attn_bwd(P[p + ".qkv"], dO, W_.p32(p + ".attn.relative_position_bias_table"), self._rel32, dqkv,
                                apart, B, sp.H, sp.W, C, nh, sp.win, sp.sft, self._mask_arg(sp))
        self._fold_bias_table(P, p, apart, R, nh, G(p + ".attn.relative_position_bias_table"))
        self._dgrad_ln_bwd(P, dqkv, W_.p16(p + ".attn.qkv.weight"), M, C, 3 * C, dxn,
                           (xin, P[p + ".mean1"], P[p + ".rstd1"], W_.p32(p + ".norm1.weight"), dx, dx, M, C,
                            G(p + ".norm1.weight"), G(p + ".norm1.bias"), p + ".1"), dict(cast=next_cast))
        self._wgrad(dqkv, 3 * C, P[p + ".xn1"], C, 3 * C, C, M, G(p + ".attn.qkv.weight"), G(p + ".attn.qkv.bias"))
        if self._lagged_hook is not None:
            fn, self._lagged_hook = self._lagged_hook, None
            fn()

    def _stage_bwd(self, P: Plan, specs: List[BlockSpec], stage_in, dx, G, have_dyb=False, next_cast=None):
        for k in reversed(range(len(specs))):
            xin = stage_in if k == 0 else P[specs[k - 1].prefix + ".out"]
            nc = self._mlp_cast(P, specs[k - 1]) if k > 0 else next_cast
            self._block_bwd(P, specs[k], xin, dx, G, have_dyb=have_dyb, next_cast=nc)
            have_dyb = True

    def _unmerge_bwd(self, P: Plan, prefix: str, s: int, dx_out, G, cast=None):
        m, W_ = self.model, self.params
        B = P.B
        H, W, C = self.grid[0] >> s, self.grid[1] >> s, m.embed_dim << s
        M = B * H * W
        dz = P[f"lvl{s}.dz2"]
        cb, cs, ct = cast if cast is not None else (None, None, 1)
        gbias = G(prefix + ".expand.bias") if m.patch_unmerging else None
        if not m.patch_unmerging:
            R = ops.expand_norm_bwd_partial_rows(B, H, W, 2)
            Cn = C // 2
            part = P.scratch("exp." + prefix, R * 3 * Cn)
            ops.expand_norm_bwd(P[f"lvl{s}.ey"], P[f"lvl{s}.emean"], P[f"lvl{s}.erstd"], W_.p32(prefix + ".norm.weight"),
                                dz, part, B, H, W, 2, Cn, dy_fine=P[f"lvl{s}.dfine"], ld=Cn)
            self._fold(part, 3 * Cn, G(prefix + ".norm.weight"), Cn, R)
            self._fold(part + 4 * Cn, 3 * Cn, G(prefix + ".norm.bias"), Cn, R)
        self._wgrad(dz, 2 * C, P[f"lvl{s}.xb"], C, 2 * C, C, M, G(prefix + ".expand.weight"), gbias)
        if s in self._glue_done:
            ops.skip_unmerge_bwd(**self._glue_done.pop(s))
            self._release_deferred()
            return
        self._gemm(dz, W_.p16(prefix + ".expand.weight"), M, C, 2 * C, lda=2 * C, ldb=C, b_trans=True, epi=EPI_F32,
                 out=dx_out, ldo=C, out2=cb, ldo2=C if cb is not None else 0, rowscale=cs, rows_per_sample=ct,
                 packed=self._pk(prefix + ".expand.weight", transposed=True))
        self._release_deferred()

    grad_overwrite = False
    adam_ctx = None
    adam_fused = frozenset()
    adam_apply = False
    adam_probe = None
    adam_sites = None
    _gflat = None
    fuse_adamw_folds = True

    def overwrite_supported(self, B: int) -> bool:
        return bool(self.group_wgrad and self.overlap_wgrad)

    def run_backward(self, P: Plan, gflat: torch.Tensor, gscale_dev=None, gscale: float = 1.0, bucket_hook=None,
                     join_tags=None, overwrite: bool = False, apply_adamw: bool = False, pack_at_end: bool = False,
                     bucket_on_side: bool = False):
        m, W_ = self.model, self.params
        B, E, nl = P.B, m.embed_dim, m.num_layers
        H0, W0 = self.grid
        self._pending, self._lagged_hook, self._deferred, self._carry = [], None, None, ()
        self._detached = None
        self._glue_done = {}
        self._pack_ev = None
        self.grad_overwrite = bool(overwrite)
        self.pack_at_end = bool(pack_at_end)
        self._gflat = gflat
        self._drop = P.drop
        self.adam_apply = bool(apply_adamw and overwrite and self.adam_ctx is not None)
        if self._loss_final is not None:
            self._side(self._loss_final)
            self._loss_final = None
        gbase = gflat.data_ptr()
        G = lambda name: gbase + 4 * W_.offset[name]
        user_hook = bucket_hook or (lambda tag: None)

        def join_and_fire(tag):
            self._wait_side()
            user_hook(tag)

        def hook(tag):
            if self._lagged_hook is not None:
                fn, self._lagged_hook = self._lagged_hook, None
                fn()
            bucket = join_tags is not None and tag in join_tags
            if bucket and bucket_on_side and tag != "embed" and self.overlap_wgrad:
                def fire(tag=tag):
                    if self._carry:
                        carry, self._carry = list(self._carry), ()
                        ops.reduce_rows_multi(carry, adam=self._adam_arg())
                    user_hook(tag)
                self._pending.append(("f", fire))
                self._flush_wgrads(mark=self.pack_at_end and self.adam_apply and tag == self._pack_mark_tag)
                return
            if bucket and self.detach_buckets and tag != "embed" and self.overlap_wgrad and self._pending:
                self._release_deferred()
                self._detached, self._pending = self._pending, []
                self._wait_side()
                user_hook(tag)
                return
            self._flush_wgrads(mark=self.pack_at_end and self.adam_apply and tag == self._pack_mark_tag)
            if tag == "embed":
                join_and_fire(tag)
            elif bucket:
                self._lagged_hook = lambda: join_and_fire(tag)
            else:
                user_hook(tag)

        M0 = B * H0 * W0
        gdw = G("decoder_pred.weight")
        if m.pixel_shuffle:
            tpart = P["tail.dwd_part"]
            head_w, head_b = "ps_head.conv_expand.0.weight", "ps_head.conv_expand.0.bias"
            targs = (P["tail.xn"], W_.p16(head_w), W_.p32(head_b), W_.p32("decoder_pred.weight"), P.pred)
            r = m.upscale_factor
            NE = r * r * E
            tkw = dict(target=P.target, gscale_dev=gscale_dev, gscale=gscale,
                       in_chans=m.in_chans, r=r)
            self._tail_fused = self.fuse_tail_bwd and ops.tail_fused_bwd_supported(E, r)
            if self._tail_fused:
                x_last = P[self.dec_blocks[-1][-1].prefix + ".out"] if nl > 1 else P[self.enc_blocks[0][-1].prefix + ".out"]
                dx0 = P["dec0.dx"] if nl > 1 else P["enc0.dx"]
                if self.fuse_tail_ln_bwd:
                    cb, cs, ct = self._mlp_cast(P, (self.dec_blocks[-1] if nl > 1 else self.enc_blocks[0])[-1]) or (None, None, 1)
                    R = (M0 + 31) // 32
                    lnp = P.scratch("lnp.norm_up.fused", R * 2 * E)
                    ops.tail_bwd_dgrad_ln(*targs, tpart, B, H0, W0, E, x_last, P["tail.mean"], P["tail.rstd"],
                                          W_.p32("norm_up.weight"), dx0, lnp, dx_bf16=cb, cast_rowscale=cs,
                                          cast_rows_per_sample=ct, **tkw)
                    self._fold(lnp, 2 * E, G("norm_up.weight"), E, R)
                    self._fold(lnp + 4 * E, 2 * E, G("norm_up.bias"), E, R)
                else:
                    ops.tail_bwd_dgrad(*targs, P["tail.dxn"], tpart, B, H0, W0, E, **tkw)
                sp = ops.tail_wgrad_splits(B, H0, W0, E, m.in_chans, r)
                nw = NE * E
                slab = P.scratch("tail.wslab", sp * (nw + NE))
                self._side_first(lambda: ops.tail_wgrad(*targs, slab, slab + 4 * sp * nw, B, H0, W0, E, **tkw))
                self._fold(slab, nw, G(head_w), nw, sp)
                self._fold(slab + 4 * sp * nw, NE, G(head_b), NE, sp)
            else:
                ops.tail_bwd(*targs, P["tail.dz"], tpart, B, H0, W0, E, **tkw)
                self._wgrad(P["tail.dz"], NE, P["tail.xn"], E, NE, E, M0, G(head_w), G(head_b))
            if m.in_chans == 1:
                self._fold(tpart, 128, gdw, E, (M0 + 31) // 32)
            else:
                for k in range(m.in_chans):
                    self._fold(tpart.data_ptr() + 4 * 128 * k, 128 * m.in_chans, gdw + 4 * E * k, E, (M0 + 31) // 32)
        else:
            r = m.upscale_factor
            NE = r * r * E
            pre = "final_patch_expanding"
            ops.l1_loss_bwd(P.pred, P.target, gscale_dev, gscale, P.dpred, P.pred.numel())
            R = ops.expand_norm_bwd_partial_rows(B, H0, W0, r)
            nrow = (2 + m.in_chans) * E
            part = P.scratch("exp.final", R * nrow)
            ops.expand_norm_bwd(P["tail.ey"], P["tail.emean"], P["tail.erstd"], W_.p32(pre + ".norm.weight"), P["tail.dz"],
                                part, B, H0, W0, r, E, dpred=P.dpred, dotw=W_.p32("decoder_pred.weight"),
                                beta=W_.p32(pre + ".norm.bias"), in_chans=m.in_chans)
            self._fold(part, nrow, G(pre + ".norm.weight"), E, R)
            self._fold(part + 4 * E, nrow, G(pre + ".norm.bias"), E, R)
            self._fold(part + 8 * E, nrow, gdw, m.in_chans * E, R)
            head_w = pre + ".expand.weight"
            self._wgrad(P["tail.dz"], NE, P["tail.xn"], E, NE, E, M0, G(head_w))
        if not (m.pixel_shuffle and self._tail_fused):
            self._gemm(P["tail.dz"], W_.p16(head_w), M0, E, NE, lda=NE, ldb=E, b_trans=True,
                     epi=EPI_BF16, out=P["tail.dxn"], ldo=E)
        x_last = P[self.dec_blocks[-1][-1].prefix + ".out"] if nl > 1 else P[self.enc_blocks[0][-1].prefix + ".out"]
        dx = P["dec0.dx"] if nl > 1 else P["enc0.dx"]
        if not (m.pixel_shuffle and self._tail_fused and self.fuse_tail_ln_bwd):
            self._ln_bwd(P, P["tail.dxn"], x_last, P["tail.mean"], P["tail.rstd"], W_.p32("norm_up.weight"), None, dx, M0,
                         E, G("norm_up.weight"), G("norm_up.bias"), "norm_up",
                         cast=self._mlp_cast(P, (self.dec_blocks[-1] if nl > 1 else self.enc_blocks[0])[-1]))
        hook("head")
        for i in reversed(range(nl - 1)):
            s = nl - i - 2
            Cs = E << s
            Ms = B * (H0 >> s) * (W0 >> s)
            dx = P[f"dec{s}.dx"]
            if i < nl - 2:
                self._unmerge_bwd(P, f"layers_up.{i}.upsample", s, dx, G,
                                  cast=self._mlp_cast(P, self.dec_blocks[i][-1]))
            dys = P[f"dec{s}.dyskip"]
            self._stage_bwd(P, self.dec_blocks[i], P[f"dec{s}.in"], dx, G, have_dyb=True,
                            next_cast=(dys, None, 1))
            pre = f"skip_connection_layers.{i}"
            self._wgrad(dys, Cs, P[f"dec{s}.cat"], 2 * Cs, Cs, 2 * Cs, Ms, G(pre + ".weight"), G(pre + ".bias"))
            if self._glue_unmerge(2 * Cs, B, H0 >> (s + 1), W0 >> (s + 1)) and self._has_copies(
                    pre + ".weight", ("first_patch_expanding" if i == 0 else f"layers_up.{i - 1}.upsample") + ".expand.weight"):
                up_blocks = self.dec_blocks[i - 1] if i > 0 else self.enc_blocks[nl - 1]
                cb, cs, ct = self._mlp_cast(P, up_blocks[-1]) or (None, None, 1)
                self._glue_done[s + 1] = dict(
                    dy_skip=dys, w_skip_t_packed=W_.p16t(pre + ".weight"), dz=P[f"lvl{s + 1}.dz2"],
                    w_expand_t_packed=W_.p16t(("first_patch_expanding" if i == 0 else f"layers_up.{i - 1}.upsample") + ".expand.weight"),
                    dx=P[f"dec{s + 1}.dx"] if i > 0 else P[f"enc{nl - 1}.dx"], dx_bf16=cb, cast_rowscale=cs,
                    cast_rows_per_sample=ct, B=B, H=H0 >> (s + 1), W=W0 >> (s + 1), C=2 * Cs)
            elif m.patch_unmerging:
                self._gemm(dys, W_.p16(pre + ".weight"), Ms, Cs, Cs, lda=Cs, ldb=2 * Cs, b_trans=True,
                           epi=EPI_UNSHUF2_BF16, out=P[f"lvl{s + 1}.dz2"], ldo=4 * Cs, psH=H0 >> (s + 1), psW=W0 >> (s + 1),
                           packed=self._pk(pre + ".weight", transposed=True))
            else:
                self._gemm(dys, W_.p16(pre + ".weight"), Ms, Cs, Cs, lda=Cs, ldb=2 * Cs, b_trans=True, epi=EPI_BF16,
                           out=P[f"lvl{s + 1}.dfine"], ldo=Cs)
            hook(f"dec{i}")
        dx = P[f"enc{nl - 1}.dx"]
        if nl > 1:
            self._unmerge_bwd(P, "first_patch_expanding", nl - 1, dx, G,
                              cast=self._mlp_cast(P, self.enc_blocks[nl - 1][-1]))
        for s in reversed(range(nl)):
            dx = P[f"enc{s}.dx"]
            bottom_to_merge = (s == nl - 1 and s > 0)
            self._stage_bwd(P, self.enc_blocks[s], P[f"enc{s}.in"], dx, G, have_dyb=(nl > 1),
                            next_cast=(P[f"enc{s}.dyb"], None, 1) if bottom_to_merge else None)
            if s > 0 and self._glue_merge_bwd(E << (s - 1), B, H0 >> (s - 1), W0 >> (s - 1)) and self._has_copies(
                    f"layers.{s - 1}.downsample.reduction.weight", *([f"skip_connection_layers.{nl - s - 2}.weight"] if s < nl - 1 else [])):
                Cp, Cs = E << (s - 1), E << s
                Hp, Wp = H0 >> (s - 1), W0 >> (s - 1)
                rows = B * (Hp // 2) * (Wp // 2)
                pre = f"layers.{s - 1}.downsample"
                has_skip = s < nl - 1
                R = ops.merge_bwd_partial_rows(Cp, B, Hp, Wp)
                part = P.scratch("lnp." + pre + ".glue", R * 8 * Cp)
                cb, cs, ct = self._mlp_cast(P, self.enc_blocks[s - 1][-1]) or (None, None, 1)
                ops.merge_bwd(dx_in=dx if has_skip else None, dy_skip=P[f"dec{s}.dyskip"] if has_skip else None,
                              w_skip_t_packed=W_.p16t(f"skip_connection_layers.{nl - s - 2}.weight") if has_skip else None,
                              dyb=P[f"enc{s}.dyb"], w_red_t_packed=W_.p16t(pre + ".reduction.weight"),
                              x_prev=P[self.enc_blocks[s - 1][-1].prefix + ".out"], mean=P[f"enc{s - 1}.mmean"],
                              rstd=P[f"enc{s - 1}.mrstd"], gamma=W_.p32(pre + ".norm.weight"), dx_prev=P[f"enc{s - 1}.dx"],
                              param_partials=part, dx_bf16=cb, cast_rowscale=cs, cast_rows_per_sample=ct, B=B, H=Hp, W=Wp, Cp=Cp)
                self._wgrad(P[f"enc{s}.dyb"], 2 * Cp, P[f"enc{s - 1}.xm"], 4 * Cp, 2 * Cp, 4 * Cp, rows, G(pre + ".reduction.weight"))
                self._fold(part, 8 * Cp, G(pre + ".norm.weight"), 4 * Cp, R)
                self._fold(part + 16 * Cp, 8 * Cp, G(pre + ".norm.bias"), 4 * Cp, R)
                hook(f"enc{s}")
                continue
            if s < nl - 1:
                Cs = E << s
                Ms = B * (H0 >> s) * (W0 >> s)
                i = nl - s - 2
                self._gemm(P[f"dec{s}.dyskip"], W_.p16(f"skip_connection_layers.{i}.weight") + 2 * Cs, Ms, Cs, Cs,
                         lda=Cs, ldb=2 * Cs, b_trans=True, epi=EPI_F32, out=dx, ldo=Cs, accumulate=True,
                         out2=P[f"enc{s}.dyb"] if s > 0 else None, ldo2=Cs if s > 0 else 0,
                         packed=self._pk(f"skip_connection_layers.{i}.weight", transposed=True, row0=Cs, K=Cs))
            if s > 0:
                Cp = E << (s - 1)
                Hp, Wp = H0 >> (s - 1), W0 >> (s - 1)
                rows = B * (Hp // 2) * (Wp // 2)
                pre = f"layers.{s - 1}.downsample"
                dyb, dxm = P[f"enc{s}.dyb"], P["t.dxm"]
                self._wgrad(dyb, 2 * Cp, P[f"enc{s - 1}.xm"], 4 * Cp, 2 * Cp, 4 * Cp, rows,
                            G(pre + ".reduction.weight"))
                self._gemm(dyb, W_.p16(pre + ".reduction.weight"), rows, 4 * Cp, 2 * Cp, lda=2 * Cp, ldb=4 * Cp,
                         b_trans=True, epi=EPI_BF16, out=dxm, ldo=4 * Cp, packed=self._pk(pre + ".reduction.weight", transposed=True))
                xprev = P[self.enc_blocks[s - 1][-1].prefix + ".out"]
                self._ln_bwd(P, dxm, xprev, P[f"enc{s - 1}.mmean"], P[f"enc{s - 1}.mrstd"], W_.p32(pre + ".norm.weight"),
                             None, P[f"enc{s - 1}.dx"], rows, 4 * Cp, G(pre + ".norm.weight"), G(pre + ".norm.bias"),
                             pre, merge=True, H=Hp, W=Wp, cast=self._mlp_cast(P, self.enc_blocks[s - 1][-1]))
            if s == 0:
                self._pending.append(("c", None))
            hook(f"enc{s}")
        kw = 8 if m.circular_padding else m.patch_size[1]
        o0 = W_.offset["patch_embed.proj.weight"]
        rel = lambda n: 4 * (W_.offset[n] - o0)
        ep = P.embed_part_ptr
        if self._drop and self._drop[0]:
            ops.dropout_scale(P["enc0.dx"], False, B * H0 * W0, E, **self._dkw(P, None, 0))
        ops.patch_embed_bwd(P.x_in, W_.p32("patch_embed.proj.weight"), W_.p32("patch_embed.proj.bias"),
                            W_.p32("patch_embed.norm.weight"), P["enc0.dx"], ep, ep + rel("patch_embed.proj.bias"),
                            ep + rel("patch_embed.norm.weight"), ep + rel("patch_embed.norm.bias"), B, m.in_chans,
                            m.img_size[0], m.img_size[1], E, m.patch_size[0], m.patch_size[1], kw, m.circular_padding,
                            self.eps, partial_stride=P.embed_stride)
        gpe, nbe = G("patch_embed.proj.weight"), ops.patch_embed_bwd_blocks(B * H0 * W0)
        embed_on_chain = self.embed_fold_on_chain and self.pack_at_end and self.adam_apply and self.overlap_wgrad
        if embed_on_chain:
            kw = dict(overwrite=self.grad_overwrite)
            if kw["overwrite"] and self.fuse_adamw_folds and self._in_gflat(gpe):
                if self.adam_probe is not None:
                    self.adam_probe[gpe] = max(P.embed_stride, self.adam_probe.get(gpe, 0))
                kw["adamw"] = self.adam_apply and gpe in self.adam_fused
                if kw["adamw"] and self.adam_sites is not None:
                    self.adam_sites[gpe] = "fold"
            ops.reduce_rows_multi([ops.reduce_region(ep, P.embed_stride, gpe, P.embed_stride, nbe, **kw)], adam=self._adam_arg())
        if self.pack_at_end and self.adam_apply and self._pack_ev is None:
            self._mark_side()
        if self._pack_ev is not None:
            torch.cuda.current_stream().wait_event(self._pack_ev)
            W_.refresh_transposes(late=False if W_.pk_late else None)
            self._pack_ev = None
        if not embed_on_chain:
            self._fold(ep, P.embed_stride, gpe, P.embed_stride, nbe)
        hook("embed")

    graph_module = knobs.on("TULIP_GRAPH_MODULE", True)

    def _module_sequence(self, P: Plan, key, fn):
        graphs = P.__dict__.setdefault("_module_graphs", {})
        key = key + (self.fuse_wide, self.fuse_wide_bwd, self.fuse_block96, self.fuse_block96_bwd, self.split_wide, self.split_wide_bwd,
                     self.fc1_grad_wide, self.fc1_grad96, self.recompute96, self.fuse_deep, self.fuse_tail_fwd, self.fuse_tail_bwd, self.fuse_glue, self.pair96, self.packed_gemm,
                     int(self._drop_seed), int(self.n_drop_slots), self.dropout_state())
        ent = graphs.get(key)
        if not self.graph_module or ent is None:
            fn()
            graphs[key] = "warm"
            return
        if ent == "warm":
            cur = torch.cuda.current_stream()
            cap = torch.cuda.Stream(device=self.device)
            cap.wait_stream(cur)
            with torch.cuda.stream(cap):
                ent = torch.cuda.CUDAGraph()
                try:
                    ent.capture_begin(capture_error_mode="thread_local")
                    fn()
                    ent.capture_end()
                except BaseException:
                    P.reset_exchange()
                    raise
            cur.wait_stream(cap)
            graphs[key] = ent
        ent.replay()

    def _module_forward(self, P: Plan):
        train = bool(self.model.training)

        def seq():
            self.params.shadow_dirty = True
            self.draw_drop_scales(P, train)
            self.run_forward(P)
        self._module_sequence(P, ("fwd", train, self.attn_fp8), seq)
        self.params.shadow_dirty = True
        P.generation += 1

    def _module_backward(self, P: Plan, dloss):
        W_ = self.params
        if not hasattr(P, "_mod_gbufs"):
            P._mod_gbufs = [torch.zeros(W_.total, dtype=torch.float32, device=self.device) for _ in range(2)]
            P._mod_gscale = torch.ones(1, dtype=torch.float32, device=self.device)
            P._mod_gidle = _storage_users(P._mod_gbufs[0])
            if P._mod_gidle >= (1 << 30) or _storage_users(P._mod_gbufs[1]) != P._mod_gidle:
                P._mod_gidle = -1
        if dloss is None:
            P._mod_gscale.fill_(1.0)
        else:
            P._mod_gscale.copy_(dloss.detach().reshape(1))
        which = next((i for i, b in enumerate(P._mod_gbufs[:2]) if _storage_users(b) == P._mod_gidle), None)
        if which is None:
            if len(P._mod_gbufs) == 2:
                P._mod_gbufs.append(torch.zeros(W_.total, dtype=torch.float32, device=self.device))
            which = 2
        g = P._mod_gbufs[which]
        over = self.overwrite_supported(P.B)
        if not over:
            g.zero_()
        self._module_sequence(P, ("bwd", self.attn_fp8, which),
                              lambda: self.run_backward(P, g, gscale_dev=P._mod_gscale, gscale=1.0, overwrite=over))
        return g.clone() if which == 2 else g

    def output_shape(self, B: int):
        r = self.model.upscale_factor
        return (B, self.model.in_chans, self.grid[0] * r, self.grid[1] * r)

    def check_target(self, B: int, target):
        want = self.output_shape(B)
        if self.model.upscale_factor != 4 and tuple(target.shape) != want:
            raise ValueError(f"target shape {tuple(target.shape)} is not the model's output shape {want} "
                             f"(batch, in_chans, token grid {self.grid} * upscale_factor {self.model.upscale_factor})")

    def autograd_forward(self, x, target, mc_drop: bool):
        self.bind(x.device)
        self.params.shadow_dirty = True
        B = x.shape[0]
        P = self.plan(B)
        P.x_in.copy_(x.reshape(P.x_in.shape).float())
        if mc_drop or target is None:
            self.draw_drop_scales(P, self.model.training)
            self.run_forward(P, with_loss=False)
            self.params.shadow_dirty = True
            return P.pred.clone()
        self.check_target(B, target)
        P.target.copy_(target.reshape(P.target.shape).float())
        params = self._cur_params if self._cur_params is not None else self.params.current_params(self.model)
        need_grad = torch.is_grad_enabled() and any(p.requires_grad for p in params)
        if not need_grad:
            self.draw_drop_scales(P, self.model.training)
            self.run_forward(P)
            self.params.shadow_dirty = True
            return P.pred.clone(), P.losses[0].clone(), P.losses[1].clone()
        return _TulipFn.apply(self, P, *params)


def _storage_users(t: torch.Tensor) -> int:
    f = getattr(torch._C, "_storage_Use_Count", None)
    return f(t.untyped_storage()._cdata) if f is not None else 1 << 30


class _TulipFn(torch.autograd.Function):

    @staticmethod
    def forward(ctx, eng: TulipEngine, P: Plan, *params):
        eng._module_forward(P)
        ctx.eng, ctx.P, ctx.gen = eng, P, P.generation
        pred, pixel = P.pred.clone(), P.losses[1].clone()
        ctx.mark_non_differentiable(pred, pixel)
        return pred, P.losses[0].clone(), pixel

    @staticmethod
    def backward(ctx, _dpred, dloss, _dpixel):
        eng, P = ctx.eng, ctx.P
        if ctx.gen != P.generation:
            raise RuntimeError("tulip_amd: backward() must follow its own forward() (activation workspaces are "
                               "reused by the next forward of the same batch size)")
        W_ = eng.params
        gflat = eng._module_backward(P, dloss)
        grads = tuple(gflat[W_.offset[n]:W_.offset[n] + W_.numel[n]].view(W_.shape[n]) for n in W_.names)
        return (None, None) + grads
```

### tulip_amd/ops.py

```python
from __future__ import annotations

import ctypes
from typing import Optional

import torch

from . import _lib
from ._lib import (EPI_BF16, EPI_F32, EPI_GELU_BWD, EPI_GELU_DUAL,
                   EPI_PIXSHUF2_F32, EPI_RESID_F32, EPI_SPLIT_F32, EPI_UNSHUF2_BF16, check)

BF16 = torch.bfloat16
F32 = torch.float32


def _p(t):
    if t is None or isinstance(t, int):
        return t
    return t.data_ptr()


def _stream():
    return torch.cuda.current_stream().cuda_stream


# ... 394 lines not shown


def dropout_scale(x, is_bf16, rows, cols, key, seed, site, p, ld=None):
    check(_lib.load().tulip_dropout_scale(_p(x), int(bool(is_bf16)), rows, cols, cols if ld is None else ld, _p(key),
                                          _seed(seed), int(site), float(p), _stream()), "tulip_dropout_scale")


def dropout_resid_ln(y, aux, rowscale, rows_per_sample, out, out_bf16, ln, eps, rows, C, key, seed, site, p):
    g, b, xn, mean, rstd = ln if ln is not None else (None,) * 5
    check(_lib.load().tulip_dropout_resid_ln(_p(y), _p(aux), _p(rowscale), rows_per_sample, _p(out), _p(out_bf16), _p(g),
                                             _p(b), _p(xn), _p(mean), _p(rstd), float(eps), rows, C, _p(key), _seed(seed),
                                             int(site), float(p), _stream()), "tulip_dropout_resid_ln")


def dropout_cast(dx, y, rows, cols, rowscale, rows_per_sample, key, seed, site, p):
    check(_lib.load().tulip_dropout_cast(_p(dx), _p(y), rows, cols, _p(rowscale), rows_per_sample, _p(key), _seed(seed),
                                         int(site), float(p), _stream()), "tulip_dropout_cast")


def window_attn_fwd_drop(qkv, bias_table, rel_index, out, B, H, W, C, nh, win, shift, masked, key, seed, site, p):
    rc = _lib.load().tulip_window_attn_fwd_drop(_p(qkv), _p(bias_table), _p(rel_index), _p(out), B, H, W, C, nh, win[0],
                                                win[1], shift[0], shift[1], int(masked), _p(key), _seed(seed), int(site),
                                                float(p), _stream())
    check(rc, "tulip_window_attn_fwd_drop")


def window_attn_bwd_drop(qkv, dout, bias_table, rel_index, dqkv, dbias_dense, B, H, W, C, nh, win, shift, masked, key, seed,
                         site, p):
    rc = _lib.load().tulip_window_attn_bwd_drop(_p(qkv), _p(dout), _p(bias_table), _p(rel_index), _p(dqkv),
                                                _p(dbias_dense), B, H, W, C, nh, win[0], win[1], shift[0], shift[1],
                                                int(masked), _p(key), _seed(seed), int(site), float(p), _stream())
    check(rc, "tulip_window_attn_bwd_drop")


def kitti_range_map(points, n, rows, cols, ang_start_y, ang_res_y, ang_res_x, max_range, min_range, winner, out):
    check(_lib.load().tulip_kitti_range_map(_p(points), n, rows, cols, float(ang_start_y), float(ang_res_y),
                                            float(ang_res_x), float(max_range), float(min_range), _p(winner), _p(out),
                                            _stream()), "tulip_kitti_range_map")


def swin96_block_fwd(stamps=None, **kw):
    d = _lib.Swin96Desc()
    for name, _t in _lib.Swin96Desc._fields_:
        v = kw.pop(name, None)
        setattr(d, name, _p(v) if name not in ("B", "H", "W", "shift_h", "shift_w", "masked", "eps") else v)
    if kw:
        raise TypeError(f"unknown fields {sorted(kw)}")
    if stamps is not None:
        check(_lib.load().tulip_swin96_block_fwd_profiled(ctypes.byref(d), _p(stamps), _stream()), "tulip_swin96_block_fwd_profiled")
        return
    check(_lib.load().tulip_swin96_block_fwd(ctypes.byref(d), _stream()), "tulip_swin96_block_fwd")


def _swin96_desc(kw):
    d = _lib.Swin96Desc()
    kw = dict(kw)
    for name, _t in _lib.Swin96Desc._fields_:
        v = kw.pop(name, None)
        setattr(d, name, _p(v) if name not in ("B", "H", "W", "shift_h", "shift_w", "masked", "eps") else v)
    if kw:
        raise TypeError(f"unknown fields {sorted(kw)}")
    return d


def swin96_pair_sync_bytes(B, H, W) -> int:
    return int(_lib.load().tulip_swin96_pair_sync_bytes(B, H, W))


def swin96_pair_fwd(first: dict, second: dict, sync):
    d0, d1 = _swin96_desc(first), _swin96_desc(second)
    check(_lib.load().tulip_swin96_pair_fwd(ctypes.byref(d0), ctypes.byref(d1), _p(sync), sync.numel() * sync.element_size(),
                                            _stream()), "tulip_swin96_pair_fwd")


def swinw_supported(C, H, W) -> bool:
    return bool(_lib.load().tulip_swinw_supported(C, H, W))


def swinw_block_fwd(C, out_bf16=None, stamps=None, exchange=None, **kw):
    d = _lib.Swin96Desc()
    for name, _t in _lib.Swin96Desc._fields_:
        v = kw.pop(name, None)
        setattr(d, name, _p(v) if name not in ("B", "H", "W", "shift_h", "shift_w", "masked", "eps") else v)
    if kw:
        raise TypeError(f"unknown fields {sorted(kw)}")
    if exchange is not None:
        check(_lib.load().tulip_swinw_block_fwd_split(ctypes.byref(d), C, _p(out_bf16), _p(exchange),
                                                      exchange.numel() * exchange.element_size(), _p(stamps), _stream()),
              "tulip_swinw_block_fwd_split")
        return
    if stamps is not None:
        check(_lib.load().tulip_swinw_block_fwd_profiled(ctypes.byref(d), C, _p(out_bf16), _p(stamps), _stream()),
              "tulip_swinw_block_fwd_profiled")
        return
    check(_lib.load().tulip_swinw_block_fwd(ctypes.byref(d), C, _p(out_bf16), _stream()), "tulip_swinw_block_fwd")


def swinw_split_bytes(C, B, H, W) -> int:
    return _lib.load().tulip_swinw_split_bytes(C, B, H, W)


def stamp_realtime(dst) -> None:
    check(_lib.load().tulip_stamp_realtime(_p(dst), _stream()), "tulip_stamp_realtime")


def swinw_bwd_partial_rows(C, B, H, W) -> int:
    return _lib.load().tulip_swinw_bwd_partial_rows(C, B, H, W)


def swinw_block_bwd(C, exchange=None, **kw):
    d = _lib.Swin96BwdDesc()
    for name, _t in _lib.Swin96BwdDesc._fields_:
        v = kw.pop(name, None)
        setattr(d, name, _p(v) if name not in ("B", "H", "W", "shift_h", "shift_w", "masked") else v)
    if kw:
        raise TypeError(f"unknown fields {sorted(kw)}")
    if exchange is not None:
        check(_lib.load().tulip_swinw_block_bwd_split(ctypes.byref(d), C, _p(exchange), exchange.numel() * exchange.element_size(),
                                                      _stream()), "tulip_swinw_block_bwd_split")
        return
    check(_lib.load().tulip_swinw_block_bwd(ctypes.byref(d), C, _stream()), "tulip_swinw_block_bwd")


def swind_supported(C, H, W, win) -> bool:
    return bool(_lib.load().tulip_swind_supported(C, H, W, int(win[0]), int(win[1])))


def swind_groups(C, B, H, W, win) -> int:
    return _lib.load().tulip_swind_groups(C, B, H, W, int(win[0]), int(win[1]))


def swind_block_fwd(C, win, out_bf16=None, phases=15, stamps=None, **kw):
    d = _lib.Swin96Desc()
    for name, _t in _lib.Swin96Desc._fields_:
        v = kw.pop(name, None)
        setattr(d, name, _p(v) if name not in ("B", "H", "W", "shift_h", "shift_w", "masked", "eps") else v)
    if kw:
        raise TypeError(f"unknown fields {sorted(kw)}")
    check(_lib.load().tulip_swind_block_fwd(ctypes.byref(d), C, int(win[0]), int(win[1]), _p(out_bf16), phases, _p(stamps),
                                            _stream()), "tulip_swind_block_fwd")


def swind_block_bwd(C, win, d_norm_out, phases=15, stamps=None, **kw):
    d = _lib.Swin96BwdDesc()
    for name, _t in _lib.Swin96BwdDesc._fields_:
        v = kw.pop(name, None)
        setattr(d, name, _p(v) if name not in ("B", "H", "W", "shift_h", "shift_w", "masked") else v)
    if kw:
        raise TypeError(f"unknown fields {sorted(kw)}")
    check(_lib.load().tulip_swind_block_bwd(ctypes.byref(d), C, int(win[0]), int(win[1]), _p(d_norm_out), phases, _p(stamps),
                                            _stream()), "tulip_swind_block_bwd")


def pack_items(entries):
    return ((_lib.PackItem * max(len(entries), 1))(*[_lib.PackItem(_p(s), _p(d), r, c, int(t)) for s, d, r, c, t in entries]),
            len(entries))


def pack_bf16_multi(items, n):
    for k in range(0, n, _lib.PACK_MAX):
        cnt = min(_lib.PACK_MAX, n - k)
        check(_lib.load().tulip_pack_bf16_multi(ctypes.byref(items, k * ctypes.sizeof(_lib.PackItem)), cnt, _stream()),
              "tulip_pack_bf16_multi")


def swin96_bwd_partial_rows(B, H, W) -> int:
    return _lib.load().tulip_swin96_bwd_partial_rows(B, H, W)


def swin96_block_bwd(stamps=None, **kw):
    d = _lib.Swin96BwdDesc()
    for name, _t in _lib.Swin96BwdDesc._fields_:
        v = kw.pop(name, None)
        setattr(d, name, _p(v) if name not in ("B", "H", "W", "shift_h", "shift_w", "masked") else v)
    if kw:
        raise TypeError(f"unknown fields {sorted(kw)}")
    if stamps is not None:
        check(_lib.load().tulip_swin96_block_bwd_profiled(ctypes.byref(d), _p(stamps), _stream()), "tulip_swin96_block_bwd_profiled")
        return
    check(_lib.load().tulip_swin96_block_bwd(ctypes.byref(d), _stream()), "tulip_swin96_block_bwd")


def _fill(cls, kw, ints):
    d = cls()
    for name, _t in cls._fields_:
        v = kw.pop(name, None)
        if name in ints:
            setattr(d, name, 0 if v is None else v)
        else:
            setattr(d, name, _p(v))
    if kw:
        raise TypeError(f"unknown fields {sorted(kw)}")
    return d


def merge_fwd_supported(Cin, B, H, W) -> bool:
    return bool(_lib.load().tulip_merge_fwd_supported(Cin, B, H, W))


def merge_fwd(**kw):
    d = _fill(_lib.MergeFwdDesc, kw, ("ld_bf16", "B", "H", "W", "Cin", "eps"))
    check(_lib.load().tulip_merge_fwd(ctypes.byref(d), _stream()), "tulip_merge_fwd")


def merge_bwd_supported(Cp, B, H, W) -> bool:
    return bool(_lib.load().tulip_merge_bwd_supported(Cp, B, H, W))


def merge_bwd_partial_rows(Cp, B, H, W) -> int:
    return _lib.load().tulip_merge_bwd_partial_rows(Cp, B, H, W)


def merge_bwd(**kw):
    d = _fill(_lib.MergeBwdDesc, kw, ("cast_rows_per_sample", "B", "H", "W", "Cp"))
    check(_lib.load().tulip_merge_bwd(ctypes.byref(d), _stream()), "tulip_merge_bwd")


def unmerge_skip_supported(C, B, H, W) -> bool:
    return bool(_lib.load().tulip_unmerge_skip_supported(C, B, H, W))


def unmerge_skip_fwd(**kw):
    d = _fill(_lib.UnmergeSkipDesc, kw, ("B", "H", "W", "C"))
    check(_lib.load().tulip_unmerge_skip_fwd(ctypes.byref(d), _stream()), "tulip_unmerge_skip_fwd")


def skip_unmerge_bwd(**kw):
    d = _fill(_lib.SkipUnmergeBwdDesc, kw, ("cast_rows_per_sample", "B", "H", "W", "C"))
    check(_lib.load().tulip_skip_unmerge_bwd(ctypes.byref(d), _stream()), "tulip_skip_unmerge_bwd")
```

Before: 4303 range-images/s.

## Fuse LayerNorm backward into deep Swin block backward kernels with norm1 hand-over

```diff
diff --git a/include/tulip_hip.h b/include/tulip_hip.h
--- a/include/tulip_hip.h
+++ b/include/tulip_hip.h
@@ -345,6 +345,9 @@
                           hipStream_t stream);
 int tulip_swind_block_bwd(const tulip_swin96_bwd_desc* d, int C, int wh, int ww, float* d_norm_out, int phases, uint64_t* stamps,
                           hipStream_t stream);
+int tulip_swind_block_bwd_ln(const tulip_swin96_bwd_desc* d, int C, int wh, int ww, float* d_norm_out, int phases, uint64_t* stamps,
+                             float* dx2, const float* next_x, const float* next_mean, const float* next_rstd,
+                             const float* next_gamma, float* next_partials, hipStream_t stream);
 
 
 typedef struct tulip_merge_fwd_desc {
diff --git a/tulip_amd/_lib.py b/tulip_amd/_lib.py
--- a/tulip_amd/_lib.py
+++ b/tulip_amd/_lib.py
@@ -98,6 +98,7 @@
     "tulip_swind_groups": [I, I, I, I, I, I],
     "tulip_swind_block_fwd": [P, I, I, I, P, I, P, P],
     "tulip_swind_block_bwd": [P, I, I, I, P, I, P, P],
+    "tulip_swind_block_bwd_ln": [P, I, I, I, P, I, P, P, P, P, P, P, P, P],
     "tulip_pack_bf16_multi": [P, I, P],
     "tulip_layernorm_fwd": [P, P, P, P, P, P, I, I, F, I, I, I, I, P],
     "tulip_layernorm_bwd": [P, P, P, P, P, P, P, I, I, I, I, I, I, P, P, P, I, P],
diff --git a/tulip_amd/csrc/swind.hip b/tulip_amd/csrc/swind.hip
--- a/tulip_amd/csrc/swind.hip
+++ b/tulip_amd/csrc/swind.hip
@@ -67,10 +67,12 @@
     bf16x8 ring[PF][NTILE];
     const bf16_t* wt[NTILE];
     static constexpr int koff(int p) { return 512 * ((p / SEG) * SEGSTRIDE + (p % SEG)); }
-    __device__ __forceinline__ void start() {
+    __device__ __forceinline__ void start() { start_steps<0, PF>(); }
+    template <int P0, int P1>
+    __device__ __forceinline__ void start_steps() {
         static_for<PF>([&](auto P_) {
             constexpr int p = decltype(P_)::value;
-            if constexpr (p < KSTEPS) {
+            if constexpr (p < KSTEPS && p >= P0 && p < P1) {
 #pragma unroll
                 for (int i = 0; i < NTILE; ++i) ring[p][i] = *(const bf16x8*)(wt[i] + koff(p));
             }
@@ -135,6 +137,10 @@
     int B, H, W, wh, ww, sh, sw, masked, save, ngrp;
     float eps, scale;
 };
+struct DeepLnArgs : DeepArgs {
+    const float *ln_dn, *ln_x, *ln_mean, *ln_rstd, *ln_gamma, *ln_dres;
+    float *ln_out, *ln_part;
+};
 #if TULIP_DEV_VARIANTS
 #define DEEP_STAMP(k) do { if (a.prof && lane == 0) a.prof[((size_t)blockIdx.x * NWV + wid) * 16 + (k)] = __builtin_amdgcn_s_memtime(); } while (0)
 #else
@@ -204,6 +210,124 @@
                 }
             }
         }
+    }
+};
+
+template <int C, int T, int NWV>
+struct LnBwdPro {
+    using RP = RowPro<C, T, NWV>;
+    static constexpr int LPT = RP::LPT, TPW = RP::TPW, NJ = RP::NJ, NP = RP::NP;
+    static constexpr int NACT = (T + TPW - 1) / TPW < NWV ? (T + TPW - 1) / TPW : NWV;
+    float4 xh[NP][NJ];
+    uint2 dpk[NP][NJ];
+    static constexpr bool LATE_RES = NWV > 8 || NP > 1;
+    float4 dv[NJ];
+    float mu, rs;
+    size_t row;
+    int tl, tt, ws;
+    static_assert(T % TPW == 0, "whole waves");
+    __device__ __forceinline__ bool active(int p) const { return (ws + p * NWV) * TPW < T; }
+    __device__ __forceinline__ void load(const DeepLnArgs& a, const TokMapD& tm, int p, int wid, int lane) {
+        ws = __builtin_amdgcn_readfirstlane(wid);
+        tl = lane % LPT;
+        tt = ws * TPW + lane / LPT + p * NWV * TPW;
+        row = tm.row(tt < T ? tt : T - 1);
+        if (active(p)) {
+#pragma unroll
+            for (int j = 0; j < NJ; ++j) {
+                const size_t off = row * C + 4 * tl + 4 * LPT * j;
+                dv[j] = *(const float4*)(a.ln_dn + off);
+                xh[p][j] = *(const float4*)(a.ln_x + off);
+            }
+            mu = a.ln_mean[row]; rs = a.ln_rstd[row];
+        }
+    }
+    static __device__ __forceinline__ float4 unpack(uint2 d) {
+        return make_float4(bf2f((bf16_t)(d.x & 0xffff)), bf2f((bf16_t)(d.x >> 16)), bf2f((bf16_t)(d.y & 0xffff)), bf2f((bf16_t)(d.y >> 16)));
+    }
+    template <int P, class EMIT>
+    __device__ __forceinline__ void pass(const DeepLnArgs& a, const float* gam, bool writer, EMIT&& emit) {
+        if (!active(P)) return;
+        constexpr int NK = 64 / LPT;
+        float s1[NK], s2[NK];
+#pragma unroll
+        for (int k = 0; k < NK; ++k) s1[k] = s2[k] = 0.f;
+#pragma unroll
+        for (int j = 0; j < NJ; ++j) {
+            const float4 ga = *(const float4*)(gam + 4 * tl + 4 * LPT * j);
+            dpk[P][j] = make_uint2(pack_bf16x2(dv[j].x, dv[j].y), pack_bf16x2(dv[j].z, dv[j].w));
+            const float4 d = unpack(dpk[P][j]), x = xh[P][j];
+            const float4 h = make_float4((x.x - mu) * rs, (x.y - mu) * rs, (x.z - mu) * rs, (x.w - mu) * rs);
+            xh[P][j] = h;
+            const float4 gy = make_float4(d.x * ga.x, d.y * ga.y, d.z * ga.z, d.w * ga.w);
+            s1[j % NK] += (gy.x + gy.y) + (gy.z + gy.w);
+            s2[j % NK] += (gy.x * h.x + gy.y * h.y) + (gy.z * h.z + gy.w * h.w);
+            if constexpr (!LATE_RES) dv[j] = *(const float4*)(a.ln_dres + row * C + 4 * tl + 4 * LPT * j);
+            if constexpr (!LATE_RES) __builtin_amdgcn_sched_barrier(0);
+        }
+#pragma unroll
+        for (int k = 0; k < NK; ++k) { s1[k] = group_sum<LPT>(s1[k]); s2[k] = group_sum<LPT>(s2[k]); }
+        float t1, t2;
+        if constexpr (NK == 4) { t1 = (s1[0] + s1[1]) + (s1[2] + s1[3]); t2 = (s2[0] + s2[1]) + (s2[2] + s2[3]); }
+        else { t1 = s1[0] + s1[1]; t2 = s2[0] + s2[1]; }
+        const float m1 = t1 * (1.0f / C);
+        const float m2 = t2 * (1.0f / C);
+#pragma unroll
+        for (int j = 0; j < NJ; ++j) asm volatile("" : "+v"(dpk[P][j].x), "+v"(dpk[P][j].y) : : "memory");
+#pragma unroll
+        for (int j = 0; j < NJ; ++j) {
+            const int c = 4 * tl + 4 * LPT * j;
+            const float4 ga = *(const float4*)(gam + c);
+            const float4 d = unpack(dpk[P][j]), h = xh[P][j];
+            const float4 gy = make_float4(d.x * ga.x, d.y * ga.y, d.z * ga.z, d.w * ga.w);
+            float4 r;
+            if constexpr (LATE_RES) r = *(const float4*)(a.ln_dres + row * C + c);
+            else r = dv[j];
+            float4 o = make_float4(rs * (gy.x - m1 - h.x * m2), rs * (gy.y - m1 - h.y * m2), rs * (gy.z - m1 - h.z * m2),
+                                   rs * (gy.w - m1 - h.w * m2));
+            o.x += r.x; o.y += r.y; o.z += r.z; o.w += r.w;
+            if (writer) *(float4*)(a.ln_out + row * C + c) = o;
+            emit(tt, row, c, o);
+            __builtin_amdgcn_sched_barrier(0);
+        }
+    }
+    template <int NTHR, int AVAIL>
+    __device__ __forceinline__ void parts(float* lds, float* out, int wid, int lane, int tid) const {
+        constexpr int NR = NACT * 2 * C * 4 <= AVAIL ? 1 : 2, RW = 2 * C / NR;
+        static_assert(NACT * RW * 4 <= AVAIL, "partial rows in LDS");
+        auto add = [](float x, float y) { return x + y; };
+        static_for<NR>([&](auto R_) {
+            constexpr int r = decltype(R_)::value;
+            if constexpr (r > 0) __syncthreads();
+            if (ws < NACT) {
+#pragma unroll
+                for (int j = 0; j < NJ; ++j) {
+#pragma unroll
+                    for (int q = (NR == 1 ? 0 : r); q <= (NR == 1 ? 1 : r); ++q) {
+                        float4 v = make_float4(0.f, 0.f, 0.f, 0.f);
+#pragma unroll
+                        for (int p = 0; p < NP; ++p) {
+                            if (p > 0 && !active(p)) continue;
+                            const float4 d = unpack(dpk[p][j]), h = xh[p][j];
+                            if (q == 0) { v.x += d.x * h.x; v.y += d.y * h.y; v.z += d.z * h.z; v.w += d.w * h.w; }
+                            else { v.x += d.x; v.y += d.y; v.z += d.z; v.w += d.w; }
+                        }
+                        if constexpr (LPT == 16) {
+                            v.x = xor16_reduce(v.x, add); v.y = xor16_reduce(v.y, add); v.z = xor16_reduce(v.z, add); v.w = xor16_reduce(v.w, add);
+                        }
+                        v.x = xor32_reduce(v.x, add); v.y = xor32_reduce(v.y, add); v.z = xor32_reduce(v.z, add); v.w = xor32_reduce(v.w, add);
+                        if (lane < LPT) *(float4*)(lds + wid * RW + (NR == 1 ? q * C : 0) + 4 * lane + 4 * LPT * j) = v;
+                    }
+                }
+            }
+            __syncthreads();
+            for (int idx = tid; idx < RW; idx += NTHR) {
+                float s = 0.f;
+#pragma unroll
+                for (int w = 0; w < NACT; ++w) s += lds[w * RW + idx];
+                out[r * RW + idx] = s;
+            }
+        });
     }
 };
 
@@ -469,11 +593,13 @@
     DEEP_STAMP(4);
 }
 
-template <int C, int G>
-__global__ __launch_bounds__((GeoD<C, G>::NT)) void deep_fc2_bwd_kernel(const DeepArgs a) {
+template <int C, int G, bool LN = false>
+__global__ __launch_bounds__((GeoD<C, G>::NT)) void deep_fc2_bwd_kernel(const std::conditional_t<LN, DeepLnArgs, DeepArgs> a) {
     using Z = GeoD<C, G>;
     constexpr int T = Z::T, KS = Z::KS, NWV = Z::NWV, HID = Z::HID, HS = Z::HS;
-    __shared__ __attribute__((aligned(16))) unsigned char smem[Z::B_SMEM];
+    using LNP = LnBwdPro<C, T, NWV>;
+    constexpr int PART_BYTES = !LN ? 0 : (Z::B_SMEM + LNP::NACT * 8 * C <= 163840 ? LNP::NACT * 8 * C : LNP::NACT * 4 * C);
+    __shared__ __attribute__((aligned(16))) unsigned char smem[Z::B_SMEM + PART_BYTES];
     unsigned char* const DY = smem;
     const int tid = threadIdx.x, lane = tid & 63, wid = tid >> 6, t = lane & 15, gq = lane >> 4;
     const int slice = blockIdx.x & (NS - 1), grp = blockIdx.x >> 3;
@@ -481,15 +607,40 @@
     const float s1v = a.ds1 ? a.ds1[tm.b] : 1.0f;
     DEEP_STAMP(0);
     RowPro<C, T, NWV> pro;
-    pro.load(a.dx, tm, wid, lane);
+    LNP ln;
+    float4 gamv;
+    if constexpr (LN) {
+        ln.load(a, tm, 0, wid, lane);
+        if (tid < C / 4) gamv = *(const float4*)(a.ln_gamma + 4 * tid);
+    } else {
+        pro.load(a.dx, tm, wid, lane);
+    }
     WS<4, KS, 3> w2s;
 #pragma unroll
     for (int i = 0; i < 4; ++i) w2s.wt[i] = wtile_ptr(a.w2, slice * (HS / 16) + 4 * wid + i, C, lane);
-    w2s.start();
+    constexpr int RING_EARLY = !LN ? 3 : (NWV > 8 || G > 1) ? 0 : 1;
+    w2s.template start_steps<0, RING_EARLY>();
     SliceWarm warm;
     warm.init(grp, a.ngrp, wid, lane, smem + Z::B_WARM);
     warm.touch<NWV>(a.w2 + (size_t)(slice * (HS / 16)) * KS * 512, 1, (HS / 16) * KS, 0);
-    pro.scaled(s1v, DY, a.dyb_m, slice == 0, wid, lane);
+    if constexpr (LN) {
+        float* const AFF = (float*)(smem + Z::B_AFF);
+        if (tid < C / 4) *(float4*)(AFF + 4 * tid) = gamv;
+        __syncthreads();
+        static_for<LNP::NP>([&](auto P_) {
+            constexpr int p = decltype(P_)::value;
+            if constexpr (p > 0) ln.load(a, tm, p, wid, lane);
+            ln.template pass<p>(a, AFF, slice == 0, [&](int tt, size_t row, int c, const float4& o) {
+                const bf16x4 pk = pack4(o.x * s1v, o.y * s1v, o.z * s1v, o.w * s1v);
+                if (slice == 0) store_late((bf16x4*)(a.dyb_m + row * C + c), pk);
+                put4<T>(DY, tt, c, pk);
+            });
+        });
+        if (slice == 0) ln.template parts<Z::NT, PART_BYTES>((float*)(smem + Z::B_SMEM), a.ln_part + (size_t)grp * (2 * C), wid, lane, tid);
+        w2s.template start_steps<RING_EARLY, 3>();
+    } else {
+        pro.scaled(s1v, DY, a.dyb_m, slice == 0, wid, lane);
+    }
     size_t rows[G];
 #pragma unroll
     for (int g = 0; g < G; ++g) rows[g] = tm.row(16 * g + t);
@@ -520,10 +671,11 @@
     DEEP_STAMP(4);
 }
 
-template <int C, int G>
-__global__ __launch_bounds__((GeoD<C, G>::NT)) void deep_attn_bwd_kernel(const DeepArgs a) {
+template <int C, int G, bool LN = false>
+__global__ __launch_bounds__((GeoD<C, G>::NT)) void deep_attn_bwd_kernel(const std::conditional_t<LN, DeepLnArgs, DeepArgs> a) {
     using Z = GeoD<C, G>;
     constexpr int T = Z::T, KS = Z::KS, KH = Z::KH, NWV = Z::NWV, HPW = Z::HPW, NH = Z::NH, NT = Z::NT;
+    using LNP = LnBwdPro<C, T, NWV>;
     __shared__ __attribute__((aligned(16))) unsigned char smem[Z::A_SMEM];
     unsigned char* const DY = smem;
     f32x4* const PX = (f32x4*)(smem + Z::A_QX);
@@ -533,15 +685,42 @@
     const TokMapD tm = make_map_d<G>(a.H, a.W, a.wh, a.ww, a.sh, a.sw, grp);
     DEEP_STAMP(0);
     RowStage<C, T, NT> st;
-    st.load(a.dyb_a, C, 0, tm, tid);
+    LNP ln;
+    float4 gamv;
+    if constexpr (LN) {
+        ln.load(a, tm, 0, wid, lane);
+        if (tid < C / 4) gamv = *(const float4*)(a.ln_gamma + 4 * tid);
+    } else {
+        st.load(a.dyb_a, C, 0, tm, tid);
+    }
     WS<2, KH, 6> wps;
 #pragma unroll
     for (int i = 0; i < 2; ++i) wps.wt[i] = wtile_ptr(a.wproj, 2 * head + i, C, lane) + 512 * (kh * KH);
-    wps.start();
+    constexpr int RING_EARLY = !LN ? 6 : (NWV > 8 || G > 1) ? 0 : 2;
+    wps.template start_steps<0, RING_EARLY>();
     SliceWarm warm;
     warm.init(grp, a.ngrp, wid, lane, smem + Z::A_WARM);
     warm.touch<NWV>(a.wproj + (size_t)(2 * slice * HPW) * KS * 512, 1, 2 * HPW * KS, 0);
-    st.store(DY, tid);
+    if constexpr (LN) {
+        float* const AFF = (float*)(smem + Z::A_AFF);
+        if (tid < C / 4) *(float4*)(AFF + 4 * tid) = gamv;
+        __syncthreads();
+        const float s0v = a.ds0 ? a.ds0[tm.b] : 1.0f;
+        static_for<LNP::NP>([&](auto P_) {
+            constexpr int p = decltype(P_)::value;
+            if constexpr (p > 0) ln.load(a, tm, p, wid, lane);
+            ln.template pass<p>(a, AFF, slice == 0, [&](int tt, size_t row, int c, const float4& o) {
+                const bf16x4 pk = pack4(o.x * s0v, o.y * s0v, o.z * s0v, o.w * s0v);
+                if (slice == 0) store_late((bf16x4*)(a.dyb_a + row * C + c), pk);
+                put4<T>(DY, tt, c, pk);
+            });
+        });
+        if (slice == 0)
+            ln.template parts<NT, Z::A_QX_BYTES + Z::A_HT_BYTES>((float*)(smem + Z::A_QX), a.ln_part + (size_t)grp * (2 * C), wid, lane, tid);
+        wps.template start_steps<RING_EARLY, 6>();
+    } else {
+        st.store(DY, tid);
+    }
     size_t rows[G];
     int lab[G];
 #pragma unroll
@@ -672,18 +851,21 @@
 }
 
 template <int C, int G>
-int launch_deep(const DeepArgs& a, int which, hipStream_t stream) {
+int launch_deep(const DeepLnArgs& l, int which, hipStream_t stream) {
+    const DeepArgs& a = l;
     const dim3 grid(a.ngrp * NS), block(GeoD<C, G>::NT);
     switch (which) {
         case 0: hipLaunchKernelGGL((deep_attn_fwd_kernel<C, G>), grid, block, 0, stream, a); break;
         case 1: hipLaunchKernelGGL((deep_fc1_fwd_kernel<C, G>), grid, block, 0, stream, a); break;
         case 2: hipLaunchKernelGGL((deep_fc2_bwd_kernel<C, G>), grid, block, 0, stream, a); break;
-        default: hipLaunchKernelGGL((deep_attn_bwd_kernel<C, G>), grid, block, 0, stream, a); break;
+        case 3: hipLaunchKernelGGL((deep_attn_bwd_kernel<C, G>), grid, block, 0, stream, a); break;
+        case 4: hipLaunchKernelGGL((deep_fc2_bwd_kernel<C, G, true>), grid, block, 0, stream, l); break;
+        default: hipLaunchKernelGGL((deep_attn_bwd_kernel<C, G, true>), grid, block, 0, stream, l); break;
     }
     TULIP_CHECK_LAUNCH();
     return TULIP_OK;
 }
-int dispatch_deep(const DeepArgs& a, int C, int G, int which, hipStream_t stream) {
+int dispatch_deep(const DeepLnArgs& a, int C, int G, int which, hipStream_t stream) {
     if (C == 768) return G == 2 ? launch_deep<768, 2>(a, which, stream) : launch_deep<768, 1>(a, which, stream);
     return launch_deep<1536, 1>(a, which, stream);
 }
@@ -722,7 +904,7 @@
     const bool all = d->xn1 && d->qkv && d->xn2 && d->fc1_pre && d->mean1 && d->rstd1 && d->mean2 && d->rstd2;
     if ((any && !all) || !d->x1 || !d->attn_out || !d->fc1_act || !d->x_in || !d->x_out) return TULIP_ERR_ARG;
     if (all && !(d->masked & TULIP_BLOCK_FC1_GRAD)) return TULIP_ERR_ARG;
-    DeepArgs a = {};
+    DeepLnArgs a = {};
     const int G = deep_g(C, d->B, d->H, d->W, wh, ww);
     a.ngrp = d->B * (d->H / wh) * (d->W / ww) / G;
     a.xin = d->x_in; a.x1 = d->x1; a.xout = d->x_out;
@@ -752,7 +934,7 @@
         if ((rc = dispatch_ns(n, C, G, 1, 0, stream))) return rc;
     }
     if (phases & 4) {
-        DeepArgs b = a;
+        DeepLnArgs b = a;
         if (b.prof) b.prof += 2 * pstride;
         if ((rc = dispatch_deep(b, C, G, 1, stream))) return rc;
     }
@@ -764,12 +946,17 @@
     return TULIP_OK;
 }
 
-extern "C" int tulip_swind_block_bwd(const tulip_swin96_bwd_desc* d, int C, int wh, int ww, float* d_norm_out, int phases,
-                                     uint64_t* stamps, hipStream_t stream) {
+struct NextNorm { const float *x, *mean, *rstd, *gamma; float* partials; };
+static int swind_block_bwd(const tulip_swin96_bwd_desc* d, int C, int wh, int ww, float* d_norm_out, int phases, uint64_t* stamps,
+                           bool ln2, float* dx2, const NextNorm* nx, hipStream_t stream) {
     if (!d || !deep_ok(C, d->B, d->H, d->W, wh, ww) || d->shift_h < 0 || d->shift_h >= d->H || d->shift_w < 0 || d->shift_w >= d->W ||
         !(phases & 15) || !(d->masked & TULIP_BLOCK_FC1_GRAD) || !d->qkv || !d->fc1_pre || !d_norm_out)
         return TULIP_ERR_ARG;
-    DeepArgs a = {};
+    if (ln2 && (phases & 4) && (!dx2 || dx2 == d->dx || !d->dx || !d->x1 || !d->mean2 || !d->rstd2 || !d->norm2_weight || !d->norm2_partials))
+        return TULIP_ERR_ARG;
+    if (nx && (phases & 1) && (!dx2 || dx2 == d->dx || !d->dx || !nx->x || !nx->mean || !nx->rstd || !nx->gamma || !nx->partials))
+        return TULIP_ERR_ARG;
+    DeepLnArgs a = {};
     const int G = deep_g(C, d->B, d->H, d->W, wh, ww);
     a.ngrp = d->B * (d->H / wh) * (d->W / ww) / G;
     a.dx = d->dx;
@@ -790,15 +977,26 @@
     n.out = a.dxn;
     const size_t pstride = (size_t)a.ngrp * NS * (C / 128) * 16;
     int rc;
-    if (phases & 1) { if ((rc = dispatch_deep(a, C, G, 2, stream))) return rc; }
+    if (phases & 1) {
+        DeepLnArgs b = a;
+        if (nx) {
+            b.ln_dn = d_norm_out; b.ln_x = nx->x; b.ln_mean = nx->mean; b.ln_rstd = nx->rstd; b.ln_gamma = nx->gamma; b.ln_dres = dx2;
+            b.ln_out = d->dx; b.ln_part = nx->partials;
+        }
+        if ((rc = dispatch_deep(b, C, G, nx ? 4 : 2, stream))) return rc;
+    }
     if (phases & 2) {
         n.in = a.dh; n.w = a.w1; n.prof = a.prof ? a.prof + pstride : nullptr;
         if ((rc = dispatch_ns(n, C, G, 4, 1, stream))) return rc;
     }
     if (phases & 4) {
-        DeepArgs b = a;
+        DeepLnArgs b = a;
         if (b.prof) b.prof += 2 * pstride;
-        if ((rc = dispatch_deep(b, C, G, 3, stream))) return rc;
+        if (ln2) {
+            b.ln_dn = d_norm_out; b.ln_x = d->x1; b.ln_mean = d->mean2; b.ln_rstd = d->rstd2; b.ln_gamma = d->norm2_weight; b.ln_dres = d->dx;
+            b.ln_out = dx2; b.ln_part = d->norm2_partials;
+        }
+        if ((rc = dispatch_deep(b, C, G, ln2 ? 5 : 3, stream))) return rc;
     }
     if (phases & 8) {
         n.in = a.dqkv; n.w = a.wqkv; n.prof = a.prof ? a.prof + 3 * pstride : nullptr;
@@ -806,3 +1004,16 @@
     }
     return TULIP_OK;
 }
+
+extern "C" int tulip_swind_block_bwd(const tulip_swin96_bwd_desc* d, int C, int wh, int ww, float* d_norm_out, int phases,
+                                     uint64_t* stamps, hipStream_t stream) {
+    return swind_block_bwd(d, C, wh, ww, d_norm_out, phases, stamps, false, nullptr, nullptr, stream);
+}
+
+extern "C" int tulip_swind_block_bwd_ln(const tulip_swin96_bwd_desc* d, int C, int wh, int ww, float* d_norm_out, int phases,
+                                        uint64_t* stamps, float* dx2, const float* next_x, const float* next_mean,
+                                        const float* next_rstd, const float* next_gamma, float* next_partials, hipStream_t stream) {
+    const NextNorm nx = {next_x, next_mean, next_rstd, next_gamma, next_partials};
+    const bool any = next_x || next_mean || next_rstd || next_gamma || next_partials;
+    return swind_block_bwd(d, C, wh, ww, d_norm_out, phases, stamps, true, dx2, any ? &nx : nullptr, stream);
+}
diff --git a/tulip_amd/engine.py b/tulip_amd/engine.py
--- a/tulip_amd/engine.py
+++ b/tulip_amd/engine.py
@@ -543,6 +543,8 @@
         return ok
 
     fuse_deep = knobs.on("TULIP_FUSE_DEEP", True)
+    deep_ln = knobs.on("TULIP_DEEP_LN", True)
+    deep_ln_handover = True
     deep_min_windows = knobs.integer("TULIP_FUSE_DEEP_MIN_WINDOWS", 32)
     deep_max_windows = knobs.integer("TULIP_FUSE_DEEP_MAX_WINDOWS", 64)
 
@@ -1324,7 +1326,7 @@
             return None
         return (P[sp.prefix + ".dyb_m"], self._ds(P, sp, 1), sp.H * sp.W)
 
-    def _block_bwd(self, P: Plan, sp: BlockSpec, xin, dx, G, have_dyb=False, next_cast=None):
+    def _block_bwd(self, P: Plan, sp: BlockSpec, xin, dx, G, have_dyb=False, next_cast=None, leave_norm1=False, take_norm1=None):
         W_ = self.params
         p = sp.prefix
         B, C, nh = P.B, sp.C, sp.nh
@@ -1333,10 +1335,16 @@
         dyb = P[p + ".dyb_m"]
         drop = self._dblock(sp)
         if self._fusable_deep(sp, B) and not drop:
-            dn = P.scratch("deep.dxn", max(P.B * q.H * q.W * q.C for q in self.blocks if self._fusable_deep(q, P.B)))
+            nmax = max(P.B * q.H * q.W * q.C for q in self.blocks if self._fusable_deep(q, P.B))
+            dn = P.scratch("deep.dxn", nmax)
             R = ops.swind_groups(C, B, sp.H, sp.W, sp.win)
             apart = P.scratch("apart." + p, R * nh * self.win_len ** 2)
             wt = W_.p16t
+            ln = self.deep_ln
+            if (leave_norm1 or take_norm1 is not None) and not ln:
+                raise ValueError("the norm1' hand-over between deep blocks needs deep_ln (its residual is the second buffer)")
+            dx2 = P.scratch("deep.dx2", nmax) if ln else None
+            part2 = P.scratch("lnp." + p + ".2d", R * 2 * C) if ln else None
             desc = dict(
                 dx=dx, x_in=xin, x1=P[p + ".x1"], qkv=P[p + ".qkv"], fc1_pre=P[p + ".h"], mean1=P[p + ".mean1"],
                 rstd1=P[p + ".rstd1"], mean2=P[p + ".mean2"], rstd2=P[p + ".rstd2"],
@@ -1346,19 +1354,33 @@
                 bias_table=W_.p32(p + ".attn.relative_position_bias_table"), rel_index=self._rel32,
                 drop_scale_attn=self._ds(P, sp, 0), drop_scale_mlp=self._ds(P, sp, 1), d_out_mlp=dyb, d_fc1_pre=dh,
                 d_out_attn=P[p + ".dyb_a"], d_qkv=dqkv, bias_partials=apart, B=B, H=sp.H, W=sp.W, shift_h=sp.sft[0],
-                shift_w=sp.sft[1], masked=self._mask_arg(sp, B))
-            ops.swind_block_bwd(C, sp.win, dn, phases=3, **desc)
+                shift_w=sp.sft[1], masked=self._mask_arg(sp, B), norm2_partials=part2)
+            if take_norm1 is not None:
+                q = take_norm1.prefix
+                part1 = P.scratch("lnp." + q + ".1d", R * 2 * C)
+                ops.swind_block_bwd_ln(C, sp.win, dn, dx2, phases=3, next_norm=(
+                    P[p + ".out"], P[q + ".mean1"], P[q + ".rstd1"], W_.p32(q + ".norm1.weight"), part1), **desc)
+                self._fold(part1, 2 * C, G(q + ".norm1.weight"), C, R)
+                self._fold(part1 + 4 * C, 2 * C, G(q + ".norm1.bias"), C, R)
+            else:
+                ops.swind_block_bwd(C, sp.win, dn, phases=3, **desc)
             self._release_deferred()
             self._wgrad(dyb, C, P[p + ".g"], Hd, C, Hd, M, G(p + ".mlp.fc2.weight"), G(p + ".mlp.fc2.bias"))
             self._wgrad(dh, Hd, P[p + ".xn2"], C, Hd, C, M, G(p + ".mlp.fc1.weight"), G(p + ".mlp.fc1.bias"))
-            self._ln_bwd(P, None, P[p + ".x1"], P[p + ".mean2"], P[p + ".rstd2"], W_.p32(p + ".norm2.weight"), dx, dx, M, C,
-                         G(p + ".norm2.weight"), G(p + ".norm2.bias"), p + ".2", cast=(P[p + ".dyb_a"], self._ds(P, sp, 0), tok),
-                         slabs=(dn, 1))
-            ops.swind_block_bwd(C, sp.win, dn, phases=12, **desc)
+            if ln:
+                ops.swind_block_bwd_ln(C, sp.win, dn, dx2, phases=12, **desc)
+                self._fold(part2, 2 * C, G(p + ".norm2.weight"), C, R)
+                self._fold(part2 + 4 * C, 2 * C, G(p + ".norm2.bias"), C, R)
+            else:
+                self._ln_bwd(P, None, P[p + ".x1"], P[p + ".mean2"], P[p + ".rstd2"], W_.p32(p + ".norm2.weight"), dx, dx, M, C,
+                             G(p + ".norm2.weight"), G(p + ".norm2.bias"), p + ".2", cast=(P[p + ".dyb_a"], self._ds(P, sp, 0), tok),
+                             slabs=(dn, 1))
+                ops.swind_block_bwd(C, sp.win, dn, phases=12, **desc)
             self._wgrad(P[p + ".dyb_a"], C, P[p + ".o"], C, C, C, M, G(p + ".attn.proj.weight"), G(p + ".attn.proj.bias"))
             self._fold_bias_table(P, p, apart, R, nh, G(p + ".attn.relative_position_bias_table"))
-            self._ln_bwd(P, None, xin, P[p + ".mean1"], P[p + ".rstd1"], W_.p32(p + ".norm1.weight"), dx, dx, M, C,
-                         G(p + ".norm1.weight"), G(p + ".norm1.bias"), p + ".1", cast=next_cast, slabs=(dn, 1))
+            if not leave_norm1:
+                self._ln_bwd(P, None, xin, P[p + ".mean1"], P[p + ".rstd1"], W_.p32(p + ".norm1.weight"), dx2 if ln else dx, dx, M, C,
+                             G(p + ".norm1.weight"), G(p + ".norm1.bias"), p + ".1", cast=next_cast, slabs=(dn, 1))
             self._wgrad(dqkv, 3 * C, P[p + ".xn1"], C, 3 * C, C, M, G(p + ".attn.qkv.weight"), G(p + ".attn.qkv.bias"))
             if self._lagged_hook is not None:
                 fn, self._lagged_hook = self._lagged_hook, None
@@ -1450,11 +1472,15 @@
             fn()
 
     def _stage_bwd(self, P: Plan, specs: List[BlockSpec], stage_in, dx, G, have_dyb=False, next_cast=None):
+        deep = lambda sp: self._fusable_deep(sp, P.B) and not self._dblock(sp)
+        took = False
         for k in reversed(range(len(specs))):
             xin = stage_in if k == 0 else P[specs[k - 1].prefix + ".out"]
             nc = self._mlp_cast(P, specs[k - 1]) if k > 0 else next_cast
-            self._block_bwd(P, specs[k], xin, dx, G, have_dyb=have_dyb, next_cast=nc)
-            have_dyb = True
+            leave = bool(k > 0 and self.deep_ln and self.deep_ln_handover and deep(specs[k]) and deep(specs[k - 1]) and nc is None)
+            kw = dict(leave_norm1=leave, take_norm1=specs[k + 1] if took else None) if (leave or took) else {}
+            self._block_bwd(P, specs[k], xin, dx, G, have_dyb=have_dyb, next_cast=nc, **kw)
+            have_dyb, took = True, leave
 
     def _unmerge_bwd(self, P: Plan, prefix: str, s: int, dx_out, G, cast=None):
         m, W_ = self.model, self.params
@@ -1735,7 +1761,7 @@
     def _module_sequence(self, P: Plan, key, fn):
         graphs = P.__dict__.setdefault("_module_graphs", {})
         key = key + (self.fuse_wide, self.fuse_wide_bwd, self.fuse_block96, self.fuse_block96_bwd, self.split_wide, self.split_wide_bwd,
-                     self.fc1_grad_wide, self.fc1_grad96, self.recompute96, self.fuse_deep, self.fuse_tail_fwd, self.fuse_tail_bwd, self.fuse_glue, self.pair96, self.packed_gemm,
+                     self.fc1_grad_wide, self.fc1_grad96, self.recompute96, self.fuse_deep, self.deep_ln, self.deep_ln_handover, self.fuse_tail_fwd, self.fuse_tail_bwd, self.fuse_glue, self.pair96, self.packed_gemm,
                      int(self._drop_seed), int(self.n_drop_slots), self.dropout_state())
         ent = graphs.get(key)
         if not self.graph_module or ent is None:
diff --git a/tulip_amd/ops.py b/tulip_amd/ops.py
--- a/tulip_amd/ops.py
+++ b/tulip_amd/ops.py
@@ -570,6 +570,18 @@
                                             _stream()), "tulip_swind_block_bwd")
 
 
+def swind_block_bwd_ln(C, win, d_norm_out, dx2, phases=15, stamps=None, next_norm=None, **kw):
+    d = _lib.Swin96BwdDesc()
+    for name, _t in _lib.Swin96BwdDesc._fields_:
+        v = kw.pop(name, None)
+        setattr(d, name, _p(v) if name not in ("B", "H", "W", "shift_h", "shift_w", "masked") else v)
+    if kw:
+        raise TypeError(f"unknown fields {sorted(kw)}")
+    nx = [_p(v) for v in next_norm] if next_norm is not None else [None] * 5
+    check(_lib.load().tulip_swind_block_bwd_ln(ctypes.byref(d), C, int(win[0]), int(win[1]), _p(d_norm_out), phases, _p(stamps),
+                                               _p(dx2), *nx, _stream()), "tulip_swind_block_bwd_ln")
+
+
 def pack_items(entries):
     return ((_lib.PackItem * max(len(entries), 1))(*[_lib.PackItem(_p(s), _p(d), r, c, int(t)) for s, d, r, c, t in entries]),
             len(entries))
```

New measurement: 4284 range-images/s. About the same (-0.5%).
